# jason-li-831202/Vehicle-CV-ADAS

Hardware: AMD Instinct MI355X
Metric: frames/sec end-to-end (detect+lane+NMS+track) per GPU; conv MFMA util % (higher is better)
Workload: dtype fp16x3

## Files before the change

include/adas_hip.h:

```cpp
#ifndef ADAS_HIP_H
#define ADAS_HIP_H
#include <stddef.h>
#include <stdint.h>

#ifdef __cplusplus
extern "C" {
#endif

typedef enum {
    ADAS_OK = 0,
    ADAS_ERR_INVALID = -1,
    ADAS_ERR_IO = -2,
    ADAS_ERR_FORMAT = -3,
    ADAS_ERR_HIP = -4,
    ADAS_ERR_CAPACITY = -5,
    ADAS_ERR_NO_DEVICE = -6
} adas_status;

const char* adas_last_error(void);
int adas_version(void);
int adas_device_count(void);
int adas_set_device(int index);
int adas_device_pci_bus_id(int index, char* out, int out_len);
int adas_malloc(void** d_ptr, size_t bytes);
int adas_free(void* d_ptr);
int adas_memcpy_h2d(void* d_dst, const void* h_src, size_t bytes);
int adas_memcpy_d2h(void* h_dst, const void* d_src, size_t bytes);
int adas_synchronize(void);
int adas_host_alloc(void** h_ptr, size_t bytes);
int adas_host_free(void* h_ptr);
typedef struct adas_timer adas_timer;
int adas_timer_create(adas_timer** out);
int adas_timer_destroy(adas_timer* t);
int adas_timer_start(adas_timer* t, void* stream);
int adas_timer_stop(adas_timer* t, void* stream);
int adas_timer_elapsed_ms(adas_timer* t, float* ms);

typedef struct adas_engine adas_engine;

#define ADAS_PREC_BF16 0
#define ADAS_PREC_FP32 1
#define ADAS_PREC_FP16 2
#define ADAS_PREC_FP16X3 3

int adas_engine_create(const char* model_path, int precision, int max_batch, adas_engine** out);
int adas_engine_destroy(adas_engine* e);
int adas_engine_input_shape(const adas_engine* e, int64_t dims[4]);
int adas_engine_num_outputs(const adas_engine* e);
int adas_engine_output_shape(const adas_engine* e, int index, int64_t dims[4], int* ndim);
const char* adas_engine_output_name(const adas_engine* e, int index);
int adas_engine_infer_host(adas_engine* e, const float* h_input_nchw, int batch, float* const* h_outputs);
int adas_engine_infer_device(adas_engine* e, const float* d_input_nchw, int batch, void* stream);
int adas_engine_accepts_packed_input(const adas_engine* e);
int adas_engine_precision(const adas_engine* e);
int adas_engine_model_io_half(const adas_engine* e);
int adas_engine_infer_device_packed(adas_engine* e, const uint16_t* d_input_nhwc4, int batch, void* stream);
const float* adas_engine_output_device(const adas_engine* e, int index);
int adas_engine_stats(const adas_engine* e, double* flops_per_frame, double* weight_bytes, int* num_layers);
int adas_engine_profile(adas_engine* e, const float* d_input_nchw, int batch, int iters, float* ms_per_layer,
                        int max_layers, int* num_layers);
int adas_engine_detect_sink_supported(const adas_engine* e);
int adas_engine_detect_sink_shape(const adas_engine* e, int32_t* layout, int32_t* num_anchors, int32_t* num_classes);
int adas_engine_set_detect_sink(adas_engine* e, float* d_best_conf, int32_t* d_best_cls);
int adas_engine_layer_info(const adas_engine* e, int layer, char* name, int name_cap, double* flops, int* kind);
int adas_engine_layer_kernel(const adas_engine* e, int layer, int batch, char* name, int name_cap);
int adas_engine_prepare(adas_engine* e, int batch);
int adas_engine_ml_info(const adas_engine* e, int batch, int32_t* n_launches, int32_t* n_layers, int32_t* n_items);
int adas_engine_ml_status(const adas_engine* e, int batch, uint32_t* error_word);
int adas_engine_launch_count(adas_engine* e, int batch);
int adas_engine_ml_counters(const adas_engine* e, int batch, int launch, uint32_t head16[16]);
typedef struct adas_ml_view {
    uint64_t buf;
    int32_t cs, coff, c, h, w;
} adas_ml_view;
typedef struct adas_ml_layer_desc {
    int32_t kernel, stride, act, res_mode, up_c, halo_bn;
    adas_ml_view x, y, res, up;
} adas_ml_layer_desc;
int adas_debug_ml_plan(const adas_ml_layer_desc* layers, int n_layers, int batch, int precision, int32_t* deps, int32_t* targets,
                       uint64_t* items, int items_cap, int32_t summary[4]);
int adas_debug_conv_route(const adas_ml_layer_desc* layer, int batch, int precision, char* name, int name_cap);
#define ADAS_PLAN_COLS 29
int adas_engine_plan(const adas_engine* e, int64_t* rows, int rows_cap, int32_t* n_ops, uint64_t* weight_bytes);
int adas_debug_engine_plan(const void* tables, size_t bytes, int precision, int max_batch, int64_t* rows, int rows_cap, int32_t* n_ops,
                           uint64_t* weight_bytes);
#define ADAS_LABEL_CAP 96
int adas_engine_schedule(const adas_engine* e, int batch, int32_t* step_of, int32_t* role, int cap, int32_t* n_ops, int32_t* n_steps);
int adas_debug_engine_schedule(const void* tables, size_t bytes, int precision, int max_batch, int batch, int32_t* step_of, int32_t* role,
                               char* labels, int cap, int32_t* n_ops, int32_t* n_steps);
int adas_engine_fetch_activation(adas_engine* e, int layer, int batch, float* h_out_nchw, int64_t dims[4]);

int adas_preprocess_yolo(const uint8_t* d_frames_bgr, int n, int src_h, int src_w, float* d_out_nchw, int dst_h,
                         int dst_w, int keep_ratio, void* stream);
int adas_preprocess_ufld(const uint8_t* d_frames_bgr, int n, int src_h, int src_w, float* d_out_nchw, int in_h,
                         int in_w, double crop_ratio, void* stream);
int adas_preprocess_yolo_packed(const uint8_t* d_frames_bgr, int n, int src_h, int src_w, uint16_t* d_out_nhwc4, int dst_h,
                                int dst_w, int keep_ratio, void* stream);
int adas_preprocess_ufld_packed(const uint8_t* d_frames_bgr, int n, int src_h, int src_w, uint16_t* d_out_nhwc4, int in_h,
                                int in_w, double crop_ratio, void* stream);
int adas_preprocess_yolo_packed_prec(const uint8_t* d_frames_bgr, int n, int src_h, int src_w, uint16_t* d_out_nhwc4, int dst_h,
                                     int dst_w, int keep_ratio, int precision, void* stream);
int adas_preprocess_ufld_packed_prec(const uint8_t* d_frames_bgr, int n, int src_h, int src_w, uint16_t* d_out_nhwc4, int in_h,
                                     int in_w, double crop_ratio, int precision, void* stream);

typedef struct adas_yolo_post adas_yolo_post;

#define ADAS_HEAD_V8 0
#define ADAS_HEAD_V5 1
#define ADAS_HEAD_V5_LITE 2
#define ADAS_NMS_REFERENCE 0
#define ADAS_NMS_GREEDY 1

typedef struct {
    int32_t layout;
    int32_t num_anchors;
    int32_t num_classes;
    int32_t nms_mode;
    double box_score;
    double iou_thr;
    int32_t pad_h, pad_w;
    double ratio_h, ratio_w;
    int32_t max_candidates;
    int32_t reserved;
} adas_yolo_post_params;

int adas_letterbox_params(int src_h, int src_w, int dst_h, int dst_w, int keep_ratio, adas_yolo_post_params* p);

int adas_yolo_post_create(const adas_yolo_post_params* p, int max_batch, adas_yolo_post** out);
int adas_yolo_post_destroy(adas_yolo_post* h);
int adas_yolo_post_set_input_size(adas_yolo_post* h, int in_h, int in_w);
int adas_yolo_post_run(adas_yolo_post* h, const float* d_head, int batch, void* stream);
int adas_yolo_post_scan_views(adas_yolo_post* h, float** d_best_conf, int32_t** d_best_cls);
int adas_yolo_post_run_prescanned(adas_yolo_post* h, const float* d_head, int batch, void* stream);
int adas_yolo_post_profile(adas_yolo_post* h, const float* d_head, int batch, int iters, float ms[2]);

typedef struct {
    int32_t n_found;
    int32_t n_candidates;
    int32_t n_keep;
    int32_t flags;
} adas_yolo_counts;
int adas_yolo_post_fetch(adas_yolo_post* h, int frame, adas_yolo_counts* counts, int32_t* cand_anchor,
                         double* cand_xywh, double* cand_conf, int32_t* cand_cls, int32_t* keep, double* det_xywh,
                         double* det_conf, int32_t* det_cls, int32_t* det_xyxy_int);
int adas_yolo_post_fetch_dets(adas_yolo_post* h, int frame, adas_yolo_counts* counts, int32_t* keep, double* det_xywh,
                              double* det_conf, int32_t* det_cls, int32_t* det_xyxy_int);
int adas_yolo_post_device_views(adas_yolo_post* h, const double** d_xyxy, const double** d_score,
                                const int32_t** d_cls, const int32_t** d_counts);
int adas_yolo_post_capacity(const adas_yolo_post* h, int* max_candidates);
int adas_yolo_post_head_shape(const adas_yolo_post* h, int32_t* layout, int32_t* num_anchors, int32_t* num_classes);

typedef struct adas_effdet_post adas_effdet_post;
typedef struct {
    double box_score;
    int32_t pad_h, pad_w;
    double ratio_h, ratio_w;
    int32_t max_boxes;
    int32_t reserved;
} adas_effdet_post_params;
int adas_effdet_post_create(const adas_effdet_post_params* p, int max_batch, adas_effdet_post** out);
int adas_effdet_post_destroy(adas_effdet_post* h);
int adas_effdet_post_run(adas_effdet_post* h, const float* d_boxes, const int32_t* d_ids, const float* d_confs,
                         const int32_t* h_counts, int batch, void* stream);
int adas_effdet_post_fetch(adas_effdet_post* h, int frame, int32_t* n_keep, float* xywh, float* conf, int32_t* class_id,
                           int32_t* xyxy_int);
typedef struct adas_effdet_tail adas_effdet_tail;
typedef struct {
    int32_t in_h, in_w;
    int32_t num_classes;
    int32_t max_candidates;
    int32_t max_det;
    int32_t reserved;
    double score_thr, iou_thr;
    double anchor_scale;
} adas_effdet_tail_params;
int adas_effdet_tail_create(const adas_effdet_tail_params* p, int max_batch, adas_effdet_tail** out);
int adas_effdet_tail_destroy(adas_effdet_tail* h);
int adas_effdet_tail_run(adas_effdet_tail* h, const float* const* d_reg , const float* const* d_cls , int batch, void* stream);
int adas_effdet_tail_fetch(adas_effdet_tail* h, int frame, int32_t* n_det, float* boxes_xyxy, int32_t* class_id, float* conf,
                           int32_t* n_candidates);
int adas_effdet_tail_device_views(adas_effdet_tail* h, const float** d_boxes, const int32_t** d_ids, const float** d_confs,
                                  const int32_t** d_counts);
int adas_preprocess_effdet(const uint8_t* d_frames_bgr, int n, int src_h, int src_w, float* d_out_nchw, int dst_h, int dst_w,
                           int keep_ratio, void* stream);

typedef struct adas_ufld_decode adas_ufld_decode;
#define ADAS_UFLD_MAX_POINTS 128

typedef struct {
    int32_t grid_row, cls_row, grid_col, cls_col;
    int32_t img_w, img_h;
    int32_t local_width;
    int32_t num_lanes;
    const double* h_row_anchor;
    const double* h_col_anchor;
} adas_ufld_params;

int adas_ufld_decode_create(const adas_ufld_params* p, int max_batch, adas_ufld_decode** out);
int adas_ufld_decode_destroy(adas_ufld_decode* h);
int adas_ufld_decode_run(adas_ufld_decode* h, const float* d_loc_row, const float* d_loc_col,
                         const float* d_exist_row, const float* d_exist_col, size_t stride_loc_row,
                         size_t stride_loc_col, size_t stride_exist_row, size_t stride_exist_col, int batch,
                         void* stream);
int adas_ufld_decode_fetch(adas_ufld_decode* h, int frame, int32_t* points, int32_t* counts, int32_t* detected);
int adas_ufld_decode_upload(adas_ufld_decode* h, int frame, const int32_t* points, const int32_t* counts, const int32_t* detected);

typedef struct {
    int32_t griding_num, cls_num_per_lane;
    int32_t cfg_img_w, cfg_img_h;
    int32_t input_w, input_h;
    int32_t src_w, src_h;
    const double* h_row_anchor;
} adas_ufld1_params;
int adas_ufld1_decode_create(const adas_ufld1_params* p, int max_batch, adas_ufld_decode** out);
int adas_ufld1_decode_set_source_size(adas_ufld_decode* h, int src_w, int src_h);
int adas_ufld_decode_kind(const adas_ufld_decode* h);
int adas_ufld_decode_expected_outputs(const adas_ufld_decode* h, int64_t dims[4][4]);
int adas_ufld1_decode_run(adas_ufld_decode* h, const float* d_out, size_t batch_stride, int batch, void* stream);

typedef struct adas_lane_geometry adas_lane_geometry;
typedef struct {
    int32_t img_h;
    int32_t bird_w, bird_h;
    int32_t adjust_lanes;
    double M[9];
} adas_lane_geometry_params;
typedef struct {
    int32_t area_status;
    int32_t n_area_left, n_area_right;
    int32_t direction;
    int32_t bird_counts[4];
    double curvature;
    double offset;
} adas_lane_geometry_result;
// ... 240 lines not shown
```

vehicle-cv-adas_amd/_lib.py:

```python
import ctypes as C
import os

import numpy as np

HERE = os.path.dirname(os.path.abspath(__file__))
LIB_PATH = os.environ.get("ADAS_LIB") or os.path.join(HERE, "libadas_hip.so")

UFLD_MAX_POINTS = 128
HEAD_V8, HEAD_V5, HEAD_V5_LITE = 0, 1, 2
NMS_REFERENCE, NMS_GREEDY = 0, 1
PREC_BF16, PREC_FP32, PREC_FP16, PREC_FP16X3 = 0, 1, 2, 3
PRECISIONS = {"bf16": PREC_BF16, "fp32": PREC_FP32, "fp16": PREC_FP16, "fp16x3": PREC_FP16X3}


class AdasError(RuntimeError):
    def __init__(self, code, msg):
        super().__init__(f"libadas_hip error {code}: {msg}")
        self.code = code


class YoloPostParams(C.Structure):
    _fields_ = [("layout", C.c_int32), ("num_anchors", C.c_int32), ("num_classes", C.c_int32), ("nms_mode", C.c_int32),
                ("box_score", C.c_double), ("iou_thr", C.c_double), ("pad_h", C.c_int32), ("pad_w", C.c_int32),
                ("ratio_h", C.c_double), ("ratio_w", C.c_double), ("max_candidates", C.c_int32), ("reserved", C.c_int32)]
# ... 9 lines not shown


class EffdetTailParams(C.Structure):
    _fields_ = [("in_h", C.c_int32), ("in_w", C.c_int32), ("num_classes", C.c_int32), ("max_candidates", C.c_int32), ("max_det", C.c_int32),
                ("reserved", C.c_int32), ("score_thr", C.c_double), ("iou_thr", C.c_double), ("anchor_scale", C.c_double)]


class UfldParams(C.Structure):
    _fields_ = [("grid_row", C.c_int32), ("cls_row", C.c_int32), ("grid_col", C.c_int32), ("cls_col", C.c_int32),
                ("img_w", C.c_int32), ("img_h", C.c_int32), ("local_width", C.c_int32), ("num_lanes", C.c_int32),
                ("h_row_anchor", C.c_void_p), ("h_col_anchor", C.c_void_p)]


class Ufld1Params(C.Structure):
    _fields_ = [("griding_num", C.c_int32), ("cls_num_per_lane", C.c_int32), ("cfg_img_w", C.c_int32), ("cfg_img_h", C.c_int32),
                ("input_w", C.c_int32), ("input_h", C.c_int32), ("src_w", C.c_int32), ("src_h", C.c_int32),
                ("h_row_anchor", C.c_void_p)]


class LaneGeometryParams(C.Structure):
    _fields_ = [("img_h", C.c_int32), ("bird_w", C.c_int32), ("bird_h", C.c_int32), ("adjust_lanes", C.c_int32), ("M", C.c_double * 9)]


class LaneGeometryResult(C.Structure):
    _fields_ = [("area_status", C.c_int32), ("n_area_left", C.c_int32), ("n_area_right", C.c_int32), ("direction", C.c_int32),
                ("bird_counts", C.c_int32 * 4), ("curvature", C.c_double), ("offset", C.c_double)]


class WarpParams(C.Structure):
    _fields_ = [("src_h", C.c_int32), ("src_w", C.c_int32), ("dst_h", C.c_int32), ("dst_w", C.c_int32)]


class BirdviewParams(C.Structure):
    _fields_ = [("img_w", C.c_int32), ("img_h", C.c_int32)]


class BirdviewState(C.Structure):
    _fields_ = [("src", C.c_float * 8), ("M", C.c_double * 9), ("M_inv", C.c_double * 9), ("M_warp", C.c_double * 9),
                ("n_updates", C.c_int32), ("n_rejected", C.c_int32)]


BIRDVIEW_MODES = {"Default": 1, "Top": 2, "Bottom": 3}


class AnalysisParams(C.Structure):
    _fields_ = [("focal", C.c_double), ("y_limit", C.c_double), ("distance_thres", C.c_double), ("offset_thres", C.c_double),
                ("curvae_thres", C.c_double), ("calib_curvae_thres", C.c_double), ("calib_frequency", C.c_int32), ("n_classes", C.c_int32),
                ("h_ref_height", C.c_void_p), ("max_points", C.c_int32), ("max_poly", C.c_int32)]


class AnalysisState(C.Structure):
    _fields_ = [("collision_msg", C.c_int32), ("offset_msg", C.c_int32), ("curvature_msg", C.c_int32), ("toggle_status", C.c_int32),
                ("transform_status", C.c_int32), ("oscillator", C.c_int32 * 2), ("counter_offset", C.c_int32), ("counter_curvae", C.c_int32),
                ("counter_birdview", C.c_int32), ("n_collision", C.c_int32), ("n_offset", C.c_int32), ("n_curvature", C.c_int32),
                ("n_nonfinite", C.c_int32), ("collision_record", C.c_double * 5), ("offset_record", C.c_double * 5),
                ("curvature_record", C.c_double * 10), ("direction_record", C.c_int32 * 10)]


class AnalysisInput(C.Structure):
    _fields_ = [("has_point", C.c_int32), ("area", C.c_int32), ("has_offset", C.c_int32), ("has_curvature", C.c_int32), ("direction", C.c_int32),
                ("reserved", C.c_int32), ("distance", C.c_double), ("offset", C.c_double), ("curvature", C.c_double)]


class AnalysisFrame(C.Structure):
    _fields_ = [("n_points", C.c_int32), ("has_collision", C.c_int32), ("collision_x", C.c_int32), ("collision_y", C.c_int32),
                ("collision_d", C.c_double), ("collision_index", C.c_int32), ("collision_msg", C.c_int32), ("offset_msg", C.c_int32),
                ("curvature_msg", C.c_int32), ("toggle_status", C.c_int32), ("transform_status", C.c_int32), ("oscillator", C.c_int32 * 2),
                ("counters", C.c_int32 * 3), ("check", C.c_int32), ("request", C.c_int32), ("flags", C.c_int32)]


ANALYSIS_INPUT_DTYPE = np.dtype([("has_point", "i4"), ("area", "i4"), ("has_offset", "i4"), ("has_curvature", "i4"), ("direction", "i4"),
                                 ("reserved", "i4"), ("distance", "f8"), ("offset", "f8"), ("curvature", "f8")])
ANALYSIS_OVERFLOW, ANALYSIS_NONFINITE, ANALYSIS_TRUNCATED = 1, 2, 4


class OverlayParams(C.Structure):
    _fields_ = [("src_h", C.c_int32), ("src_w", C.c_int32), ("bird_h", C.c_int32), ("bird_w", C.c_int32), ("lane_radius", C.c_int32),
                ("distance_radius", C.c_int32), ("bird_radius", C.c_int32), ("reserved", C.c_int32), ("lane_alpha", C.c_double),
                ("area_alpha", C.c_double), ("lane_colors", (C.c_uint8 * 3) * 4), ("offset_color", C.c_uint8 * 3), ("area_color", C.c_uint8 * 3),
                ("collision_colors", (C.c_uint8 * 3) * 4), ("distance_color", C.c_uint8 * 3), ("pad", C.c_uint8 * 7)]


OVERLAY_LANES, OVERLAY_AREA, OVERLAY_DISTANCE, OVERLAY_BIRD = 1, 2, 4, 8
OVERLAY_STAGES = {"lanes": OVERLAY_LANES, "area": OVERLAY_AREA, "distance": OVERLAY_DISTANCE, "bird": OVERLAY_BIRD}
OVERLAY_POLY_RANGE = 1


class BytetrackParams(C.Structure):
    _fields_ = [("track_thresh", C.c_double), ("match_thresh", C.c_double), ("frame_rate", C.c_double),
                ("track_buffer", C.c_int32), ("max_tracks", C.c_int32), ("max_dets", C.c_int32), ("reserved", C.c_int32)]


class TrackHeader(C.Structure):
    _fields_ = [("frame_id", C.c_int32), ("id_count", C.c_int32), ("n_tracked", C.c_int32), ("n_lost", C.c_int32),
                ("err", C.c_int32), ("pad", C.c_int32 * 3)]


class PipelineDesc(C.Structure):
    _fields_ = [("detector", C.c_void_p), ("lane", C.c_void_p), ("post", C.c_void_p), ("decode", C.c_void_p),
                ("tracker", C.c_void_p), ("n_streams", C.c_int32), ("use_graph", C.c_int32), ("geometry", C.c_void_p),
                ("micro_batch", C.c_int32), ("reserved", C.c_int32)]


class MlView(C.Structure):
    _fields_ = [("buf", C.c_uint64), ("cs", C.c_int32), ("coff", C.c_int32), ("c", C.c_int32), ("h", C.c_int32), ("w", C.c_int32)]


class MlLayerDesc(C.Structure):
    _fields_ = [("kernel", C.c_int32), ("stride", C.c_int32), ("act", C.c_int32), ("res_mode", C.c_int32), ("up_c", C.c_int32), ("halo_bn", C.c_int32),
                ("x", MlView), ("y", MlView), ("res", MlView), ("up", MlView)]


TRACK_DTYPE = np.dtype([("tlwh", "f8", 4), ("score", "f8"), ("track_id", "i4"), ("state", "i4"), ("is_activated", "i4"),
                        ("class_id", "i4"), ("frame_id", "i4"), ("start_frame", "i4"), ("tracklet_len", "i4"), ("traj_len", "i4")])
TRAJECTORY_LEN = 30

_P = C.c_void_p
_SIGS = {
    "adas_last_error": (C.c_char_p, []),
    "adas_version": (C.c_int, []),
    "adas_device_count": (C.c_int, []),
    "adas_set_device": (C.c_int, [C.c_int]),
    "adas_device_pci_bus_id": (C.c_int, [C.c_int, C.c_char_p, C.c_int]),
    "adas_malloc": (C.c_int, [C.POINTER(_P), C.c_size_t]),
    "adas_free": (C.c_int, [_P]),
    "adas_memcpy_h2d": (C.c_int, [_P, _P, C.c_size_t]),
    "adas_memcpy_d2h": (C.c_int, [_P, _P, C.c_size_t]),
    "adas_synchronize": (C.c_int, []),
    "adas_host_alloc": (C.c_int, [C.POINTER(_P), C.c_size_t]),
    "adas_host_free": (C.c_int, [_P]),
    "adas_timer_create": (C.c_int, [C.POINTER(_P)]),
    "adas_timer_destroy": (C.c_int, [_P]),
    "adas_timer_start": (C.c_int, [_P, _P]),
    "adas_timer_stop": (C.c_int, [_P, _P]),
    "adas_timer_elapsed_ms": (C.c_int, [_P, C.POINTER(C.c_float)]),
    "adas_engine_create": (C.c_int, [C.c_char_p, C.c_int, C.c_int, C.POINTER(_P)]),
    "adas_engine_destroy": (C.c_int, [_P]),
    "adas_engine_input_shape": (C.c_int, [_P, C.POINTER(C.c_int64)]),
    "adas_engine_num_outputs": (C.c_int, [_P]),
    "adas_engine_output_shape": (C.c_int, [_P, C.c_int, C.POINTER(C.c_int64), C.POINTER(C.c_int)]),
    "adas_engine_output_name": (C.c_char_p, [_P, C.c_int]),
    "adas_engine_infer_host": (C.c_int, [_P, _P, C.c_int, C.POINTER(_P)]),
    "adas_engine_infer_device": (C.c_int, [_P, _P, C.c_int, _P]),
    "adas_engine_accepts_packed_input": (C.c_int, [_P]),
    "adas_engine_precision": (C.c_int, [_P]),
    "adas_engine_prepare": (C.c_int, [_P, C.c_int]),
    "adas_engine_ml_info": (C.c_int, [_P, C.c_int, C.POINTER(C.c_int32), C.POINTER(C.c_int32), C.POINTER(C.c_int32)]),
    "adas_engine_ml_status": (C.c_int, [_P, C.c_int, C.POINTER(C.c_uint32)]),
    "adas_engine_launch_count": (C.c_int, [_P, C.c_int]),
    "adas_engine_ml_counters": (C.c_int, [_P, C.c_int, C.c_int, C.POINTER(C.c_uint32)]),
    "adas_debug_ml_plan": (C.c_int, [C.POINTER(MlLayerDesc), C.c_int, C.c_int, C.c_int, C.POINTER(C.c_int32), C.POINTER(C.c_int32), C.POINTER(C.c_uint64),
                                     C.c_int, C.POINTER(C.c_int32)]),
    "adas_debug_conv_route": (C.c_int, [C.POINTER(MlLayerDesc), C.c_int, C.c_int, C.c_char_p, C.c_int]),
    "adas_engine_plan": (C.c_int, [_P, C.POINTER(C.c_int64), C.c_int, C.POINTER(C.c_int32), C.POINTER(C.c_uint64)]),
    "adas_debug_engine_plan": (C.c_int, [C.c_char_p, C.c_size_t, C.c_int, C.c_int, C.POINTER(C.c_int64), C.c_int, C.POINTER(C.c_int32), C.POINTER(C.c_uint64)]),
    "adas_engine_schedule": (C.c_int, [_P, C.c_int, C.POINTER(C.c_int32), C.POINTER(C.c_int32), C.c_int, C.POINTER(C.c_int32), C.POINTER(C.c_int32)]),
    "adas_debug_engine_schedule": (C.c_int, [C.c_char_p, C.c_size_t, C.c_int, C.c_int, C.c_int, C.POINTER(C.c_int32), C.POINTER(C.c_int32), C.c_char_p,
                                             C.c_int, C.POINTER(C.c_int32), C.POINTER(C.c_int32)]),
    "adas_engine_model_io_half": (C.c_int, [_P]),
    "adas_engine_infer_device_packed": (C.c_int, [_P, _P, C.c_int, _P]),
    "adas_engine_output_device": (_P, [_P, C.c_int]),
    "adas_engine_stats": (C.c_int, [_P, C.POINTER(C.c_double), C.POINTER(C.c_double), C.POINTER(C.c_int)]),
    "adas_engine_profile": (C.c_int, [_P, _P, C.c_int, C.c_int, _P, C.c_int, C.POINTER(C.c_int)]),
    "adas_engine_layer_info": (C.c_int, [_P, C.c_int, C.c_char_p, C.c_int, C.POINTER(C.c_double), C.POINTER(C.c_int)]),
    "adas_engine_layer_kernel": (C.c_int, [_P, C.c_int, C.c_int, C.c_char_p, C.c_int]),
    "adas_engine_fetch_activation": (C.c_int, [_P, C.c_int, C.c_int, _P, C.POINTER(C.c_int64)]),
    "adas_preprocess_yolo": (C.c_int, [_P, C.c_int, C.c_int, C.c_int, _P, C.c_int, C.c_int, C.c_int, _P]),
    "adas_preprocess_ufld": (C.c_int, [_P, C.c_int, C.c_int, C.c_int, _P, C.c_int, C.c_int, C.c_double, _P]),
    "adas_preprocess_yolo_packed": (C.c_int, [_P, C.c_int, C.c_int, C.c_int, _P, C.c_int, C.c_int, C.c_int, _P]),
    "adas_preprocess_ufld_packed": (C.c_int, [_P, C.c_int, C.c_int, C.c_int, _P, C.c_int, C.c_int, C.c_double, _P]),
    "adas_preprocess_yolo_packed_prec": (C.c_int, [_P, C.c_int, C.c_int, C.c_int, _P, C.c_int, C.c_int, C.c_int, C.c_int, _P]),
    "adas_preprocess_ufld_packed_prec": (C.c_int, [_P, C.c_int, C.c_int, C.c_int, _P, C.c_int, C.c_int, C.c_double, C.c_int, _P]),
    "adas_letterbox_params": (C.c_int, [C.c_int, C.c_int, C.c_int, C.c_int, C.c_int, C.POINTER(YoloPostParams)]),
    "adas_yolo_post_create": (C.c_int, [C.POINTER(YoloPostParams), C.c_int, C.POINTER(_P)]),
    "adas_yolo_post_destroy": (C.c_int, [_P]),
    "adas_yolo_post_set_input_size": (C.c_int, [_P, C.c_int, C.c_int]),
    "adas_yolo_post_run": (C.c_int, [_P, _P, C.c_int, _P]),
    "adas_yolo_post_profile": (C.c_int, [_P, _P, C.c_int, C.c_int, C.POINTER(C.c_float)]),
    "adas_yolo_post_fetch": (C.c_int, [_P, C.c_int, C.POINTER(YoloCounts)] + [_P] * 9),
    "adas_yolo_post_fetch_dets": (C.c_int, [_P, C.c_int, C.POINTER(YoloCounts)] + [_P] * 5),
    "adas_yolo_post_device_views": (C.c_int, [_P] + [C.POINTER(_P)] * 4),
    "adas_yolo_post_scan_views": (C.c_int, [_P, C.POINTER(_P), C.POINTER(_P)]),
    "adas_yolo_post_run_prescanned": (C.c_int, [_P, _P, C.c_int, _P]),
    "adas_engine_detect_sink_supported": (C.c_int, [_P]),
    "adas_engine_detect_sink_shape": (C.c_int, [_P, C.POINTER(C.c_int32), C.POINTER(C.c_int32), C.POINTER(C.c_int32)]),
    "adas_engine_set_detect_sink": (C.c_int, [_P, _P, _P]),
    "adas_pipeline_detect_sink": (C.c_int, [_P]),
    "adas_yolo_post_capacity": (C.c_int, [_P, C.POINTER(C.c_int)]),
    "adas_yolo_post_head_shape": (C.c_int, [_P, C.POINTER(C.c_int32), C.POINTER(C.c_int32), C.POINTER(C.c_int32)]),
    "adas_effdet_post_create": (C.c_int, [C.POINTER(EffdetPostParams), C.c_int, C.POINTER(_P)]),
    "adas_effdet_post_destroy": (C.c_int, [_P]),
    "adas_effdet_post_run": (C.c_int, [_P, _P, _P, _P, _P, C.c_int, _P]),
    "adas_effdet_post_fetch": (C.c_int, [_P, C.c_int, C.POINTER(C.c_int32), _P, _P, _P, _P]),
    "adas_effdet_tail_create": (C.c_int, [C.POINTER(EffdetTailParams), C.c_int, C.POINTER(_P)]),
    "adas_effdet_tail_destroy": (C.c_int, [_P]),
    "adas_effdet_tail_run": (C.c_int, [_P, _P, _P, C.c_int, _P]),
    "adas_effdet_tail_fetch": (C.c_int, [_P, C.c_int, C.POINTER(C.c_int32), _P, _P, _P, C.POINTER(C.c_int32)]),
    "adas_effdet_tail_device_views": (C.c_int, [_P, C.POINTER(_P), C.POINTER(_P), C.POINTER(_P), C.POINTER(_P)]),
    "adas_preprocess_effdet": (C.c_int, [_P, C.c_int, C.c_int, C.c_int, _P, C.c_int, C.c_int, C.c_int, _P]),
    "adas_ufld_decode_create": (C.c_int, [C.POINTER(UfldParams), C.c_int, C.POINTER(_P)]),
    "adas_ufld_decode_destroy": (C.c_int, [_P]),
    "adas_ufld_decode_run": (C.c_int, [_P, _P, _P, _P, _P, C.c_size_t, C.c_size_t, C.c_size_t, C.c_size_t, C.c_int, _P]),
    "adas_ufld_decode_fetch": (C.c_int, [_P, C.c_int, _P, _P, _P]),
    "adas_ufld_decode_upload": (C.c_int, [_P, C.c_int, _P, _P, _P]),
    "adas_ufld1_decode_create": (C.c_int, [C.POINTER(Ufld1Params), C.c_int, C.POINTER(_P)]),
    "adas_ufld1_decode_set_source_size": (C.c_int, [_P, C.c_int, C.c_int]),
    "adas_ufld_decode_kind": (C.c_int, [_P]),
    "adas_ufld_decode_expected_outputs": (C.c_int, [_P, C.POINTER(C.c_int64)]),
    "adas_ufld1_decode_run": (C.c_int, [_P, _P, C.c_size_t, C.c_int, _P]),
    "adas_lane_geometry_create": (C.c_int, [C.POINTER(LaneGeometryParams), C.c_int, C.POINTER(_P)]),
    "adas_lane_geometry_destroy": (C.c_int, [_P]),
    "adas_lane_geometry_set_matrix": (C.c_int, [_P, _P]),
    "adas_lane_geometry_run": (C.c_int, [_P, _P, C.c_int, C.c_int, _P]),
    "adas_lane_geometry_fetch": (C.c_int, [_P, C.c_int, C.POINTER(LaneGeometryResult), _P, _P]),
    "adas_lane_geometry_run_matrices": (C.c_int, [_P, _P, C.c_int, C.c_int, _P, _P]),
    "adas_warp_run_device_matrices": (C.c_int, [_P, _P, _P, _P, C.c_int, _P]),
    "adas_birdview_create": (C.c_int, [C.POINTER(BirdviewParams), C.c_int, C.c_int, C.POINTER(_P)]),
    "adas_birdview_destroy": (C.c_int, [_P]),
    "adas_birdview_reset": (C.c_int, [_P, C.c_int]),
    "adas_birdview_request": (C.c_int, [_P, C.c_int, C.c_int, _P]),
    "adas_birdview_run": (C.c_int, [_P, _P, C.c_int, C.c_int, _P]),
    "adas_birdview_fetch_stream": (C.c_int, [_P, C.c_int, C.POINTER(BirdviewState)]),
    "adas_birdview_fetch_frame": (C.c_int, [_P, C.c_int, _P, _P, C.POINTER(C.c_int32)]),
    "adas_birdview_pending": (C.c_int, [_P, C.c_int, C.POINTER(C.c_int32)]),
    "adas_birdview_device_views": (C.c_int, [_P, C.POINTER(_P), C.POINTER(_P)]),
    "adas_pipeline_attach_birdview": (C.c_int, [_P, _P, _P]),
    "adas_pipeline_attach_analysis": (C.c_int, [_P, _P]),
    "adas_lane_geometry_device_views": (C.c_int, [_P, C.POINTER(_P), C.POINTER(_P), C.POINTER(_P), C.POINTER(C.c_int32)]),
    "adas_analysis_default_params": (C.c_int, [C.POINTER(AnalysisParams)]),
    "adas_analysis_create": (C.c_int, [C.POINTER(AnalysisParams), C.c_int, C.c_int, C.POINTER(_P)]),
    "adas_analysis_destroy": (C.c_int, [_P]),
    "adas_analysis_reset": (C.c_int, [_P, C.c_int]),
    "adas_analysis_run": (C.c_int, [_P, _P, _P, _P, C.c_int, C.c_int, _P]),
    "adas_analysis_run_arrays": (C.c_int, [_P, _P, _P, _P, C.c_int, _P, C.c_int, _P, _P, _P, C.c_int, C.c_int, _P]),
    "adas_analysis_run_inputs": (C.c_int, [_P, _P, C.c_int, C.c_int, _P]),
    "adas_analysis_fetch_stream": (C.c_int, [_P, C.c_int, C.POINTER(AnalysisState)]),
    "adas_analysis_fetch_frame": (C.c_int, [_P, C.c_int, C.POINTER(AnalysisFrame)]),
    "adas_analysis_fetch_points": (C.c_int, [_P, C.c_int, _P, _P, C.c_int]),
    "adas_pipeline_request_transform": (C.c_int, [_P, C.c_int, C.c_int]),
    "adas_overlay_default_params": (C.c_int, [C.POINTER(OverlayParams)]),
    "adas_overlay_create": (C.c_int, [C.POINTER(OverlayParams), C.c_int, C.POINTER(_P)]),
    "adas_overlay_destroy": (C.c_int, [_P]),
    "adas_overlay_set_style": (C.c_int, [_P, C.POINTER(OverlayParams)]),
    "adas_overlay_run": (C.c_int, [_P, _P, _P, _P, _P, _P, _P, C.c_int, C.c_int, C.c_int, _P]),
    "adas_overlay_run_arrays": (C.c_int, [_P, _P, _P, _P, _P, _P, C.c_int, _P, _P, _P, _P, _P, C.c_int, _P, _P, _P, _P, C.c_int, C.c_int, _P]),
    "adas_overlay_fetch": (C.c_int, [_P, C.c_int, _P]),
    "adas_overlay_device_view": (C.c_int, [_P, C.POINTER(_P)]),
    "adas_overlay_fetch_flags": (C.c_int, [_P, C.c_int, C.POINTER(C.c_int32)]),
    "adas_pipeline_attach_overlay": (C.c_int, [_P, _P]),
    "adas_pipeline_set_overlay_stages": (C.c_int, [_P, C.c_int]),
    "adas_warp_create": (C.c_int, [C.POINTER(WarpParams), C.c_int, C.POINTER(_P)]),
    "adas_warp_destroy": (C.c_int, [_P]),
    "adas_warp_set_matrix": (C.c_int, [_P, C.c_int, _P, C.c_int]),
    "adas_warp_run": (C.c_int, [_P, _P, _P, C.c_int, _P]),
    "adas_warp_fetch": (C.c_int, [_P, C.c_int, _P]),
    "adas_warp_device_view": (C.c_int, [_P, C.POINTER(_P)]),
    "adas_bytetrack_create": (C.c_int, [C.POINTER(BytetrackParams), C.c_int, C.POINTER(_P)]),
    "adas_bytetrack_destroy": (C.c_int, [_P]),
    "adas_bytetrack_reset": (C.c_int, [_P, C.c_int]),
    "adas_bytetrack_update_host": (C.c_int, [_P, C.c_int, _P, _P, _P, C.c_int]),
    "adas_bytetrack_update_device": (C.c_int, [_P, _P, _P, _P, _P, C.c_int, C.c_int, C.c_int, C.c_int, _P]),
    "adas_bytetrack_update_device_frames": (C.c_int, [_P, _P, _P, _P, _P, C.c_int, C.c_int, C.c_int, C.c_int, C.c_int, _P]),
    "adas_bytetrack_fetch": (C.c_int, [_P, C.c_int, C.POINTER(TrackHeader), _P, C.c_int]),
    "adas_bytetrack_fetch_trajectories": (C.c_int, [_P, C.c_int, _P, _P, C.c_int, C.POINTER(C.c_int32)]),
    "adas_bytetrack_reserve_frames": (C.c_int, [_P, C.c_int, C.c_int]),
    "adas_bytetrack_fetch_frame": (C.c_int, [_P, C.c_int, C.c_int, C.POINTER(TrackHeader), _P, C.c_int]),
    "adas_pipeline_create": (C.c_int, [C.POINTER(PipelineDesc), C.POINTER(_P)]),
    "adas_pipeline_destroy": (C.c_int, [_P]),
    "adas_pipeline_step": (C.c_int, [_P, _P, _P]),
    "adas_pipeline_step_frames": (C.c_int, [_P, _P, C.c_int, C.c_int, C.c_double]),
    "adas_pipeline_step_frames_host": (C.c_int, [_P, _P, C.c_int, C.c_int, C.c_double]),
    "adas_pipeline_wait_upload": (C.c_int, [_P]),
    "adas_pipeline_sync": (C.c_int, [_P]),
    "adas_pipeline_timings": (C.c_int, [_P, C.POINTER(C.c_float)]),
}

_lib = None


def exported_symbols():
    return sorted(_SIGS)


def lib():
    global _lib
    if _lib is None:
        if not os.path.exists(LIB_PATH):
            raise RuntimeError(f"{LIB_PATH} is not built; run `python vehicle-cv-adas_amd/build.py` "
                               "(hipcc --offload-arch=gfx950). There is no CPU fallback.")
        L = C.CDLL(LIB_PATH)
        for name, (res, args) in _SIGS.items():
            fn = getattr(L, name)
            fn.restype = res
            fn.argtypes = args
        _lib = L
    return _lib


def check(code):
    if code != 0:
        raise AdasError(code, lib().adas_last_error().decode("utf-8", "replace"))
    return code


def ptr(a):
    return None if a is None else a.ctypes.data_as(C.c_void_p)
# ... 92 lines not shown
```

vehicle-cv-adas_amd/csrc/conv_halo8_x3.hip:

```cpp
#include "kernels.h"
#include "elem16.h"
#include <stdlib.h>
#include <string.h>
#include <type_traits>

namespace adas {

typedef __attribute__((ext_vector_type(4))) float yf32x4;
typedef __attribute__((ext_vector_type(4))) uint32_t yu32x4;
typedef __attribute__((ext_vector_type(2))) uint32_t yu32x2;
typedef __attribute__((address_space(3))) void* ylds_vp;

struct H8XDev {
    const void* in;
    const void* wgt;
    const float* bias;
    void* out;
    const void* res;
    uint32_t in_bytes, wgt_bytes, out_bytes, res_bytes;
    int in_cs, in_coff, cin, H, W;
    int out_cs, out_coff, cout;
    int res_cs, res_coff, res_mode;
    int nck;
    int SW, NS, TPS, WW;
    uint32_t mg_ww, mg_sw;
    uint32_t mg_img, mg_tps, mg_upt;
    int ntiles, tiles8, ncb, cpw;
};

constexpr int X8_THR = 512;
constexpr int X8_BM = 256;
constexpr int X8_MAXPIX = 640;
constexpr int X8_WIN = X8_MAXPIX * 64;
constexpr int X8_TAP = 2 * 64 * 64;
constexpr int X8_WR = 2 * X8_WIN;
constexpr int X8_LDS = X8_WR + 9 * X8_TAP;
constexpr int X8_NWP = X8_MAXPIX / 16 / 8;
constexpr int X8_SLAB = 9 * 64 * 64;
constexpr uint32_t X8_OOB = 0xF0000000u;
constexpr int X8_SLOTS = 32;

__host__ __device__ constexpr int x8_look(int mode) { return mode == 2 ? 6 : 4; }

template <int N>
__device__ __forceinline__ void x8_wait_vm() {
    asm volatile("s_waitcnt vmcnt(%0)" ::"n"(N) : "memory");
}

template <int ACT>
__device__ __forceinline__ float x8_act(float v) {
    if (ACT == ACT_SILU) return x3_silu(v);
    if (ACT == ACT_RELU) return fmaxf(v, 0.0f);
    if (ACT == ACT_LEAKY) return fmaxf(v, 0.1f * v);
    return v;
}

typedef __attribute__((ext_vector_type(2))) float yf32x2;
template <int ACT>
__device__ __forceinline__ yf32x2 x8_act2(yf32x2 v) {
    if (ACT == ACT_RELU) return __builtin_elementwise_max(v, yf32x2{0.0f, 0.0f});
    return yf32x2{x8_act<ACT>(v[0]), x8_act<ACT>(v[1])};
}
__device__ __forceinline__ yf32x2 x8_join2(uint32_t h, uint32_t l) {
    return __builtin_convertvector(__builtin_bit_cast(e_f16x2, l), yf32x2) * kX3Down + __builtin_convertvector(__builtin_bit_cast(e_f16x2, h), yf32x2);
}
__device__ __forceinline__ void x8_hi_mode(bool flush) {
    if (flush) __builtin_amdgcn_s_setreg((unsigned short)(1 | (6 << 6) | (1 << 11)), 0u);
    else __builtin_amdgcn_s_setreg((unsigned short)(1 | (6 << 6) | (1 << 11)), 3u);
}
__device__ __forceinline__ uint32_t x8_cvt_hi2(yf32x2 v) {
    uint32_t h;
    asm volatile("v_cvt_pk_f16_f32 %0, %1, %2" : "=v"(h) : "v"(v[0]), "v"(v[1]));
    return h;
}
__device__ __forceinline__ uint32_t x8_lo2(yf32x2 v, uint32_t h) {
    const yf32x2 d = (v - __builtin_convertvector(__builtin_bit_cast(e_f16x2, h), yf32x2)) * kX3Up;
    return __builtin_bit_cast(uint32_t, __builtin_convertvector(d, e_f16x2));
}

__host__ __device__ constexpr int x8_issued(int k) { return 1 + ((k >= 1 && k <= X8_NWP) ? 1 : 0); }
__host__ __device__ constexpr int x8_allow(int mode, int k) {
    return mode == 2 ? x8_issued(k) + x8_issued(k - 1) + x8_issued(k - 2)
                     : x8_issued(k) + x8_issued((k + 8) % 9) + x8_issued((k + 7) % 9);
}
#ifndef ADAS_H8X_RES_TAP
#define ADAS_H8X_RES_TAP 0
#endif
constexpr int X8_RES_TAP = ADAS_H8X_RES_TAP;
#ifdef ADAS_H8X_NARROW_ST
constexpr int X8_NBIAS = 2, X8_NRES = 16;
#else
constexpr int X8_NBIAS = 2, X8_NRES = 8;
#endif

#ifdef ADAS_H8X_PROF
__device__ unsigned long long g_h8x_prof[256][32];
#define H8XP(i)                                     \
    if (lane == 0 && grp == 0) {                    \
        const unsigned long long t__ = clock64();   \
        pacc__[i] += t__ - tprev__;                 \
        tprev__ = t__;                              \
    }
#else
#define H8XP(i)
#endif

__host__ __device__ constexpr int x8s_issued(bool lo, int k, int nwp) { return ((lo ? k >= 3 : (k >= 0 && k < 3)) ? 1 : 0) + ((k >= 1 && k <= nwp) ? 1 : 0); }
__host__ __device__ constexpr int x8s_allow(bool lo, int k, int nwp) { return x8s_issued(lo, k, nwp) + x8s_issued(lo, k - 1, nwp) + x8s_issued(lo, k - 2, nwp); }

template <int ACT, int MODE, bool LH, bool SH, int NWP>
__global__ __launch_bounds__(X8_THR, 1) void conv_h8x3_kernel(H8XDev a) {
    static_assert(!SH || (MODE == 2 && !LH), "shared weight tiles: one barrier per tap row, whole tiles");
    static_assert(NWP >= 1 && NWP <= X8_NWP && (SH || NWP == X8_NWP), "window pieces per wave");
    Fp16::enter();
    typedef Fp16::vec8 hvec8;
    constexpr int LOOK = x8_look(MODE);
    extern __shared__ __attribute__((aligned(16))) uint8_t lds8[];

    const int tid = threadIdx.x, lane = tid & 63;
    const int wave = __builtin_amdgcn_readfirstlane(tid >> 6);
    const int lrow = lane & 15, kg = lane >> 4;
    const int hb = wave >> 2, grp = wave & 3;
    const int xcd = blockIdx.x & 7, slot = blockIdx.x >> 3, nslot = gridDim.x >> 3;
    int tiles_here = a.ntiles - xcd * a.tiles8;
    tiles_here = tiles_here < 0 ? 0 : (tiles_here > a.tiles8 ? a.tiles8 : tiles_here);
    const int upt = a.ncb / a.cpw;
    const int units_here = tiles_here * upt;
    if (slot >= units_here) return;

    __amdgpu_buffer_rsrc_t rin = __builtin_amdgcn_make_buffer_rsrc((void*)a.in, 0, a.in_bytes, 0x00020000);
    __amdgpu_buffer_rsrc_t rwg = __builtin_amdgcn_make_buffer_rsrc((void*)a.wgt, 0, a.wgt_bytes, 0x00020000);
    __amdgpu_buffer_rsrc_t rout = __builtin_amdgcn_make_buffer_rsrc((void*)a.out, 0, a.out_bytes, 0x00020000);
    __amdgpu_buffer_rsrc_t rres = __builtin_amdgcn_make_buffer_rsrc((void*)(a.res_mode != RES_NONE ? a.res : a.out), 0,
                                                                    a.res_mode != RES_NONE ? a.res_bytes : 0u, 0x00020000);
    const int per_img = a.NS * a.TPS;
    const int gsw[4] = {0, 2, 3, 1};
    const uint32_t wlane = (uint32_t)((lane >> 2) * 64 + (((lane & 3) ^ gsw[(lane >> 4) & 3]) << 4));
    const uint32_t wpiece = (uint32_t)((lane & 3) ^ (((lane >> 4) & 1) << 1)) << 5;
    const uint32_t wrd = (uint32_t)(X8_WR + hb * 4096 + lrow * 64 + ((kg ^ gsw[(lrow >> 2) & 3]) << 4));
    const uint32_t wlane_h = (uint32_t)((lane >> 2) * 64 + (((lane & 3) ^ gsw[(((lane >> 4) & 1) + 2 * (grp & 1)) & 3]) << 4));
    const uint32_t wdst_h = (uint32_t)(X8_WR + hb * 4096 + 2048 + grp * 512);
#ifdef ADAS_H8X_NARROW_ST
    const uint32_t ch_lane = (uint32_t)((hb * 4 + (kg >> 1)) * 32 + (kg & 1) * 8);
#else
    const uint32_t ch_lane = (uint32_t)((hb * 4 + (kg >> 1)) * 32 + (kg & 1) * 16);
#endif
    const bool has_res = a.res_mode != RES_NONE;

    struct Tile {
        int img, sx0, p0, y_first;
    };
    auto decode = [&](int u) {
        Tile t;
        int tile = xcd * a.tiles8 + (upt == 1 ? u : (int)__umulhi((uint32_t)u, a.mg_upt));
        t.img = per_img == 1 ? tile : (int)__umulhi((uint32_t)tile, a.mg_img);
        tile -= t.img * per_img;
        const int strip = a.TPS == 1 ? tile : (int)__umulhi((uint32_t)tile, a.mg_tps);
        t.sx0 = strip * a.SW;
        t.p0 = (tile - strip * a.TPS) * X8_BM;
        t.y_first = (int)(((uint32_t)t.p0 * a.mg_sw) >> 20);
        return t;
    };
    auto win_offset = [&](const Tile& t, int i) {
        const int y_lastp = (int)(((uint32_t)(t.p0 + X8_BM - 1) * a.mg_sw) >> 20);
        const int npix = (y_lastp - t.y_first + 3) * a.WW;
        const int pix = (wave + 8 * i) * 16 + (lane >> 2);
        const int wy = (int)(((uint32_t)pix * a.mg_ww) >> 20), wx = pix - wy * a.WW;
        const int iy = t.y_first - 1 + wy, ix = t.sx0 - 1 + wx;
        const bool ok = pix < npix && (unsigned)iy < (unsigned)a.H && (unsigned)ix < (unsigned)a.W;
        const uint32_t off = ((uint32_t)((t.img * a.H + iy) * a.W + ix) * (uint32_t)a.in_cs + (uint32_t)a.in_coff) * 4u + wpiece;
        const uint32_t m = 0u - (uint32_t)ok;
        return (off & m) | (X8_OOB & ~m);
    };
    auto tap00 = [&](const Tile& t, int j) {
        const int p = t.p0 + (grp * 4 + j) * 16 + lrow;
        const int y = (int)(((uint32_t)p * a.mg_sw) >> 20), xs = p - y * a.SW;
        return (uint32_t)((((y - t.y_first) * a.WW + xs) << 6) | (kg << 4));
    };
    auto tap_offset = [&](uint32_t ap64, int t) {
        const uint32_t v = ap64 + (uint32_t)(((t / 3) * a.WW + (t % 3)) << 6);
        return v ^ ((v >> 3) & 0x20u);
    };
    auto out_pixel = [&](const Tile& t, int j) {
        const int p = t.p0 + (grp * 4 + j) * 16 + lrow;
        const int y = (int)(((uint32_t)p * a.mg_sw) >> 20), x = t.sx0 + (p - y * a.SW);
        return (y < a.H && x < a.W) ? (uint32_t)((t.img * a.H + y) * a.W + x) : X8_OOB;
    };
    auto wgt_base = [&](int cb) { return (uint32_t)(((2 * cb + hb) * a.nck) * X8_SLAB + grp * 1024); };
    auto load_bias = [&](int cb, float4* b) {
#pragma unroll
        for (int i = 0; i < 2; ++i) b[i] = *reinterpret_cast<const float4*>(a.bias + cb * 64 + hb * 32 + i * 16 + kg * 4);
    };

    auto first_cb = [&](int u) { return upt == 1 ? 0 : (u - (int)__umulhi((uint32_t)u, a.mg_upt) * upt) * a.cpw; };
    int ti = slot, cb = first_cb(slot), cbi = 0;
    Tile cur = decode(ti);
    uint32_t gcur[X8_NWP], gnxt[X8_NWP];
    uint32_t xoff[4][9];
    uint32_t po[4];
#pragma unroll
    for (int i = 0; i < NWP; ++i) gcur[i] = win_offset(cur, i);
#pragma unroll
    for (int j = 0; j < 4; ++j) {
        const uint32_t ap64 = tap00(cur, j);
#pragma unroll
        for (int t = 0; t < 9; ++t) xoff[j][t] = tap_offset(ap64, t);
        po[j] = out_pixel(cur, j);
    }
    uint32_t wcur = wgt_base(cb);
    int par = 0;
    float4 biasn[2];
    load_bias(cb, biasn);

#pragma unroll
    for (int i = 0; i < NWP; ++i)
        __builtin_amdgcn_raw_ptr_buffer_load_lds(rin, (ylds_vp)(lds8 + (wave + 8 * i) * 1024), 16, gcur[i], 0, 0, 0);
#pragma unroll
    for (int t = 0; t < LOOK; ++t)
        __builtin_amdgcn_raw_ptr_buffer_load_lds(rwg, (ylds_vp)(lds8 + X8_WR + t * X8_TAP + wave * 1024), 16, wlane, wcur + t * 4096, 0, 0);
    yf32x4 acc[4][4];
#pragma unroll
    for (int j = 0; j < 4; ++j) {
#pragma unroll
        for (int i = 0; i < 2; ++i) {
            acc[i][j] = yf32x4{biasn[i].x, biasn[i].y, biasn[i].z, biasn[i].w};
            acc[i + 2][j] = yf32x4{0.f, 0.f, 0.f, 0.f};
        }
    }
    x8_wait_vm<0>();
    __builtin_amdgcn_s_barrier();
    if (MODE == 1 && hb) __builtin_amdgcn_s_barrier();
#ifdef ADAS_H8X_PROF
    unsigned long long tprev__ = clock64();
    unsigned long long pacc__[16] = {0, 0, 0, 0, 0, 0, 0, 0, 0, 0, 0, 0, 0, 0, 0, 0};
    int nit__ = 0;
#endif

    for (;;) {
        H8XP(0)
        const bool newtile = cbi + 1 == a.cpw;
        const bool has_next = !newtile || ti + nslot < units_here;
        const int cbn = newtile ? first_cb(has_next ? ti + nslot : ti) : cb + 1;
        const uint32_t ch0 = (uint32_t)(cb * 256) + ch_lane;
#ifndef ADAS_H8X_NO_TRIM
        const bool wave_on = cb * 64 + hb * 32 < a.cout;
#else
        constexpr bool wave_on = true;
#endif
        Tile nxt = cur;
        uint32_t wnxt_item = 0, apn[4] = {0, 0, 0, 0};
        yu32x4 rraw[4][2];

        auto chunk = [&](auto last_c, auto lo_c, const int c) {
            constexpr bool lastc = decltype(last_c)::value;
            constexpr bool islo = decltype(lo_c)::value;
            if (lastc) {
                if (newtile && has_next) nxt = decode(ti + nslot);
                if (!has_next) nxt.y_first = a.H + 4;
                wnxt_item = wgt_base(cbn);
#pragma unroll
                for (int j = 0; j < 4; ++j) apn[j] = tap00(nxt, j);
            } else {
#pragma unroll
                for (int i = 0; i < NWP; ++i) gcur[i] += islo ? 112u : 16u;
            }
            const uint32_t wthis = wcur + (uint32_t)c * X8_SLAB;
            const uint32_t wnext = lastc ? wnxt_item : wthis + X8_SLAB;
            const uint32_t winr = (uint32_t)(((par + c) & 1) * X8_WIN), winw = X8_WIN - winr;
            auto tap = [&](auto kk_c) {
                constexpr int kk = decltype(kk_c)::value;
                if (lastc && kk == X8_RES_TAP) load_bias(cbn, biasn);
                if (lastc && kk == X8_RES_TAP && has_res) {
#pragma unroll
                    for (int j = 0; j < 4; ++j) {
                        const uint32_t ro = po[j] == X8_OOB ? X8_OOB : (po[j] * (uint32_t)a.res_cs + (uint32_t)a.res_coff) * 4u + ch0;
#pragma unroll
                        for (int i = 0; i < 2; ++i) {
#ifdef ADAS_H8X_NARROW_ST
                            const uint32_t ri = (cb * 64 + hb * 32 + i * 16 + kg * 4 < a.cout) ? ro + i * 64 : X8_OOB;
                            const yu32x2 rh = __builtin_bit_cast(yu32x2, __builtin_amdgcn_raw_buffer_load_b64(rres, ri, 0, 0));
                            const yu32x2 rl = __builtin_bit_cast(yu32x2, __builtin_amdgcn_raw_buffer_load_b64(rres, ri + 16, 0, 0));
                            rraw[j][i] = yu32x4{rh.x, rh.y, rl.x, rl.y};
#else
                            const uint32_t ri = (cb * 64 + hb * 32 + i * 16 + (kg >> 1) * 8 < a.cout) ? ro + i * 64 : X8_OOB;
                            rraw[j][i] = __builtin_bit_cast(yu32x4, __builtin_amdgcn_raw_buffer_load_b128(rres, ri, 0, 0));
#endif
                        }
                    }
                }
                hvec8 wf[4], xf[4];
                if (wave_on) {
#pragma unroll
                    for (int i = islo ? 2 : 0; i < 4; ++i) wf[i] = *reinterpret_cast<const hvec8*>(lds8 + wrd + kk * X8_TAP + ((SH && islo) ? i - 2 : i) * 1024);
#pragma unroll
                    for (int j = 0; j < 4; ++j) xf[j] = *reinterpret_cast<const hvec8*>(lds8 + xoff[j][kk] + winr);
                }
                if constexpr (SH) {
                    if constexpr (islo ? kk >= 3 : kk < 3) {
                        constexpr int kt = (kk + 6) % 9;
                        const uint32_t src = (islo ? wnext : wthis) + (uint32_t)kt * 4096u;
                        __builtin_amdgcn_raw_ptr_buffer_load_lds(rwg, (ylds_vp)(lds8 + X8_WR + kt * X8_TAP + wave * 1024), 16, wlane, src, 0, 0);
                    }
                } else {
                    constexpr int kt = (kk + LOOK) % 9;
                    constexpr bool tgt_lo = (kk + LOOK < 9) ? islo : !islo;
                    const uint32_t src = (kk + LOOK < 9 ? wthis : wnext) + (uint32_t)kt * 4096u;
                    if (LH && tgt_lo) {
                        if (lane < 32)
                            __builtin_amdgcn_raw_ptr_buffer_load_lds(rwg, (ylds_vp)(lds8 + wdst_h + kt * X8_TAP), 16, wlane_h, src + 2048u - (uint32_t)grp * 512u, 0, 0);
                    } else {
                        __builtin_amdgcn_raw_ptr_buffer_load_lds(rwg, (ylds_vp)(lds8 + X8_WR + kt * X8_TAP + wave * 1024), 16, wlane, src, 0, 0);
                    }
                }
                if constexpr (kk >= 1 && kk <= NWP)
                    __builtin_amdgcn_raw_ptr_buffer_load_lds(rin, (ylds_vp)(lds8 + winw + (wave + 8 * (kk - 1)) * 1024), 16, lastc ? gnxt[kk - 1] : gcur[kk - 1], 0, 0, 0);
                constexpr bool sync_here = MODE != 2 || kk % 3 == 2;
                constexpr int allow = SH ? x8s_allow(islo, kk, NWP) : x8_allow(MODE, kk);
                constexpr bool with_res = kk >= X8_RES_TAP && (MODE == 2 ? kk / 3 == X8_RES_TAP / 3 : kk < X8_RES_TAP + 3);
                auto counted_wait = [&]() {
                    if (sync_here && (c > 0 || kk >= 3)) {
                        if (lastc && with_res && has_res) x8_wait_vm<allow + X8_NBIAS + X8_NRES>();
                        else if (lastc && with_res) x8_wait_vm<allow + X8_NBIAS>();
                        else x8_wait_vm<allow>();
                    }
                };
#ifndef ADAS_H8X_WAIT_LAST
                counted_wait();
#else
                if (MODE == 1) counted_wait();
#endif
                if (MODE == 1) {
                    __builtin_amdgcn_sched_barrier(0);
                    __builtin_amdgcn_s_barrier();
                    __builtin_amdgcn_sched_barrier(0);
                }
                __builtin_amdgcn_s_setprio(1);
                if (lastc) {
#pragma unroll
                    for (int j = 0; j < 4; ++j) xoff[j][kk] = tap_offset(apn[j], kk);
                    if constexpr (kk < NWP) gnxt[kk] = win_offset(nxt, kk);
                }
                if (wave_on) {
#pragma unroll
                    for (int i = islo ? 2 : 0; i < 4; ++i)
#pragma unroll
                        for (int j = 0; j < 4; ++j) acc[i][j] = Fp16::mfma(wf[i], xf[j], acc[i][j]);
                }
                if (lastc) {
#pragma unroll
                    for (int g = 0; g < (islo ? 8 : 16); ++g) {
                        __builtin_amdgcn_sched_group_barrier(0x008, 1, 0);
                        __builtin_amdgcn_sched_group_barrier(0x006, 6, 0);
                    }
                }
                __builtin_amdgcn_s_setprio(0);
                if (sync_here) {
                    __builtin_amdgcn_sched_barrier(0);
#ifdef ADAS_H8X_WAIT_LAST
                    if (MODE != 1) counted_wait();
#endif
                    __builtin_amdgcn_s_barrier();
                    __builtin_amdgcn_sched_barrier(0);
                }
            };
            tap(std::integral_constant<int, 0>{}); tap(std::integral_constant<int, 1>{}); tap(std::integral_constant<int, 2>{});
            tap(std::integral_constant<int, 3>{}); tap(std::integral_constant<int, 4>{}); tap(std::integral_constant<int, 5>{});
            tap(std::integral_constant<int, 6>{}); tap(std::integral_constant<int, 7>{}); tap(std::integral_constant<int, 8>{});
#ifdef ADAS_H8X_PROF
            if (lastc) { H8XP(3) } else if (islo) { H8XP(2) } else { H8XP(1) }
#endif
        };
        for (int c = 0; c + 1 < a.nck; ++c) {
            if (c & 1) chunk(std::false_type{}, std::true_type{}, c);
            else chunk(std::false_type{}, std::false_type{}, c);
        }
        chunk(std::true_type{}, std::true_type{}, a.nck - 1);

        __builtin_amdgcn_s_waitcnt(0x0F70);
        H8XP(4)
#if !defined(ADAS_H8X_SCALAR_EPI) && !defined(ADAS_H8X_NARROW_ST)
        auto write_out = [&](auto rm_c) {
            constexpr int RM = decltype(rm_c)::value;
            yf32x2 val[4][2][2];
#pragma unroll
            for (int j = 0; j < 4; ++j)
#pragma unroll
                for (int i = 0; i < 2; ++i) {
                    yf32x2 v0 = yf32x2{acc[i + 2][j][0], acc[i + 2][j][1]} * kX3Down + yf32x2{acc[i][j][0], acc[i][j][1]};
                    yf32x2 v1 = yf32x2{acc[i + 2][j][2], acc[i + 2][j][3]} * kX3Down + yf32x2{acc[i][j][2], acc[i][j][3]};
                    if (RM != RES_NONE) {
                        const auto q0 = __builtin_amdgcn_permlane16_swap(rraw[j][i].x, rraw[j][i].z, false, false);
                        const auto q1 = __builtin_amdgcn_permlane16_swap(rraw[j][i].y, rraw[j][i].w, false, false);
                        const yf32x2 r0 = x8_join2(q0[0], q0[1]), r1 = x8_join2(q1[0], q1[1]);
                        if (RM == RES_BEFORE_ACT) { v0 = x8_act2<ACT>(v0 + r0); v1 = x8_act2<ACT>(v1 + r1); }
                        else { v0 = x8_act2<ACT>(v0) + r0; v1 = x8_act2<ACT>(v1) + r1; }
                    } else {
                        v0 = x8_act2<ACT>(v0); v1 = x8_act2<ACT>(v1);
                    }
                    val[j][i][0] = v0; val[j][i][1] = v1;
                    acc[i][j] = yf32x4{biasn[i].x, biasn[i].y, biasn[i].z, biasn[i].w};
                    acc[i + 2][j] = yf32x4{0.f, 0.f, 0.f, 0.f};
                }
            uint32_t hw[4][2][2];
            x8_hi_mode(true);
#pragma unroll
            for (int j = 0; j < 4; ++j)
#pragma unroll
                for (int i = 0; i < 2; ++i) {
                    hw[j][i][0] = x8_cvt_hi2(val[j][i][0]);
                    hw[j][i][1] = x8_cvt_hi2(val[j][i][1]);
                }
            x8_hi_mode(false);
#pragma unroll
            for (int j = 0; j < 4; ++j) {
                const uint32_t oo = po[j] == X8_OOB ? X8_OOB : (po[j] * (uint32_t)a.out_cs + (uint32_t)a.out_coff) * 4u + ch0;
#pragma unroll
                for (int i = 0; i < 2; ++i) {
                    const uint32_t oi = (cb * 64 + hb * 32 + i * 16 + (kg >> 1) * 8 < a.cout) ? oo + i * 64 : X8_OOB;
                    const uint32_t l0 = x8_lo2(val[j][i][0], hw[j][i][0]), l1 = x8_lo2(val[j][i][1], hw[j][i][1]);
                    const auto s0 = __builtin_amdgcn_permlane16_swap(hw[j][i][0], l0, false, false);
                    const auto s1 = __builtin_amdgcn_permlane16_swap(hw[j][i][1], l1, false, false);
                    __builtin_amdgcn_raw_buffer_store_b128(yu32x4{s0[0], s1[0], s0[1], s1[1]}, rout, oi, 0, 0);
                }
            }
        };
#else
        auto write_out = [&](auto rm_c) {
            constexpr int RM = decltype(rm_c)::value;
#pragma unroll
            for (int j = 0; j < 4; ++j) {
                const uint32_t oo = po[j] == X8_OOB ? X8_OOB : (po[j] * (uint32_t)a.out_cs + (uint32_t)a.out_coff) * 4u + ch0;
#pragma unroll
                for (int i = 0; i < 2; ++i) {
#ifdef ADAS_H8X_NARROW_ST
                    const uint32_t oi = (cb * 64 + hb * 32 + i * 16 + kg * 4 < a.cout) ? oo + i * 64 : X8_OOB;
#else
                    const uint32_t oi = (cb * 64 + hb * 32 + i * 16 + (kg >> 1) * 8 < a.cout) ? oo + i * 64 : X8_OOB;
#endif
                    float v[4];
#pragma unroll
                    for (int e = 0; e < 4; ++e) v[e] = acc[i][j][e] + acc[i + 2][j][e] * kX3Down;
                    if (RM != RES_NONE) {
#ifdef ADAS_H8X_NARROW_ST
                        const uint32_t wh0 = rraw[j][i].x, wh1 = rraw[j][i].y, wl0 = rraw[j][i].z, wl1 = rraw[j][i].w;
#else
                        const auto q0 = __builtin_amdgcn_permlane16_swap(rraw[j][i].x, rraw[j][i].z, false, false);
                        const auto q1 = __builtin_amdgcn_permlane16_swap(rraw[j][i].y, rraw[j][i].w, false, false);
                        const uint32_t wh0 = q0[0], wl0 = q0[1], wh1 = q1[0], wl1 = q1[1];
#endif
                        const e_f16x2 h0 = __builtin_bit_cast(e_f16x2, wh0);
                        const e_f16x2 h1 = __builtin_bit_cast(e_f16x2, wh1);
                        const e_f16x2 l0 = __builtin_bit_cast(e_f16x2, wl0);
                        const e_f16x2 l1 = __builtin_bit_cast(e_f16x2, wl1);
                        const float r[4] = {x3_join(h0[0], l0[0]), x3_join(h0[1], l0[1]), x3_join(h1[0], l1[0]), x3_join(h1[1], l1[1])};
#pragma unroll
                        for (int e = 0; e < 4; ++e) v[e] = RM == RES_BEFORE_ACT ? x8_act<ACT>(v[e] + r[e]) : x8_act<ACT>(v[e]) + r[e];
                    } else {
#pragma unroll
                        for (int e = 0; e < 4; ++e) v[e] = x8_act<ACT>(v[e]);
                    }
                    e_f16x2 h0, h1, l0, l1;
                    _Float16 h, l;
                    x3_split(v[0], h, l); h0[0] = h; l0[0] = l;
                    x3_split(v[1], h, l); h0[1] = h; l0[1] = l;
                    x3_split(v[2], h, l); h1[0] = h; l1[0] = l;
                    x3_split(v[3], h, l); h1[1] = h; l1[1] = l;
#ifdef ADAS_H8X_NARROW_ST
                    __builtin_amdgcn_raw_buffer_store_b64(yu32x2{__builtin_bit_cast(uint32_t, h0), __builtin_bit_cast(uint32_t, h1)}, rout, oi, 0, 0);
                    __builtin_amdgcn_raw_buffer_store_b64(yu32x2{__builtin_bit_cast(uint32_t, l0), __builtin_bit_cast(uint32_t, l1)}, rout, oi + 16, 0, 0);
#else
                    {
                        const auto s0 = __builtin_amdgcn_permlane16_swap(__builtin_bit_cast(uint32_t, h0), __builtin_bit_cast(uint32_t, l0), false, false);
                        const auto s1 = __builtin_amdgcn_permlane16_swap(__builtin_bit_cast(uint32_t, h1), __builtin_bit_cast(uint32_t, l1), false, false);
                        __builtin_amdgcn_raw_buffer_store_b128(yu32x4{s0[0], s1[0], s0[1], s1[1]}, rout, oi, 0, 0);
                    }
#endif
                    acc[i][j] = yf32x4{biasn[i].x, biasn[i].y, biasn[i].z, biasn[i].w};
                    acc[i + 2][j] = yf32x4{0.f, 0.f, 0.f, 0.f};
                }
            }
        };
#endif
        if (a.res_mode == RES_NONE) write_out(std::integral_constant<int, RES_NONE>{});
        else if (a.res_mode == RES_BEFORE_ACT) write_out(std::integral_constant<int, RES_BEFORE_ACT>{});
        else write_out(std::integral_constant<int, RES_AFTER_ACT>{});
        H8XP(5)
#ifdef ADAS_H8X_PROF
        ++nit__;
#endif

        if (!has_next) break;
        if (newtile) {
            ti += nslot;
            cur = nxt;
#pragma unroll
            for (int j = 0; j < 4; ++j) po[j] = out_pixel(cur, j);
        }
        cb = cbn;
        cbi = newtile ? 0 : cbi + 1;
#pragma unroll
        for (int i = 0; i < NWP; ++i) gcur[i] = gnxt[i];
        wcur = wnxt_item;
        par = (par + a.nck) & 1;
    }
    if (MODE == 1 && !hb) __builtin_amdgcn_s_barrier();
#ifdef ADAS_H8X_PROF
    if (lane == 0 && grp == 0) {
        unsigned long long* b__ = g_h8x_prof[blockIdx.x & 255];
        for (int i__ = 0; i__ < 16; ++i__)
            if (i__ != 7) atomicAdd(&b__[i__ + 16 * hb], pacc__[i__]);
        atomicAdd(&b__[7 + 16 * hb], (unsigned long long)nit__);
    }
#endif
}

#ifdef ADAS_H8X_PROF
extern "C" int adas_debug_h8x_prof(unsigned long long* out32, int reset) {
    static unsigned long long h[256][32];
    if (out32) {
        if (hipMemcpyFromSymbol(h, HIP_SYMBOL(g_h8x_prof), sizeof(h)) != hipSuccess) return -1;
        for (int i = 0; i < 32; ++i) {
            out32[i] = 0;
            for (int b = 0; b < 256; ++b) out32[i] += h[b][i];
        }
    }
    if (reset) {
        memset(h, 0, sizeof(h));
        if (hipMemcpyToSymbol(HIP_SYMBOL(g_h8x_prof), h, sizeof(h)) != hipSuccess) return -1;
    }
    return 0;
}
#endif

static int x8_mode() {
    static int v = -1;
    if (v < 0) {
        const char* e = getenv("ADAS_HALO8_X3");
        v = e ? atoi(e) : 1;
    }
    return v;
}

static int x8_policy() {
    static int v = -1;
    if (v < 0) {
        const char* e = getenv("ADAS_H8X_PLAN");
        v = e ? atoi(e) : 1;
    }
    return v;
}
static bool x8_plan(int Ho, int Wo, HaloPlan* pl) { return plan_halo(Ho, Wo, 1, pl, X8_MAXPIX, 0, x8_policy()); }

static double x8_min_fill() {
    static double v = -1.0;
    if (v < 0) { const char* e = getenv("ADAS_H8X_MIN_FILL"); v = e ? atof(e) : 0.6; if (!(v > 0.0 && v <= 1.0)) v = 0.6; }
    return v;
}
static int x8_blocks_per_unit(long tiles8, int ncb) {
    for (int cpw = ncb; cpw >= 1; --cpw) {
        if (ncb % cpw) continue;
        const long units8 = tiles8 * (ncb / cpw), rounds = (units8 + X8_SLOTS - 1) / X8_SLOTS;
        if (units8 >= X8_SLOTS && (double)units8 / (double)(rounds * X8_SLOTS) >= x8_min_fill()) return cpw;
    }
    if (tiles8 * ncb >= 12 && tiles8 * ncb < X8_SLOTS) return 1;
    return 0;
}

static int x8_cin_pad(int cin) { return (cin + 31) / 32 * 32; }
static int x8_cout_pad(int cout) { return (cout + 63) / 64 * 64; }
bool halo8_x3_shape_ok(int kh, int kw, int stride, int pad, const TView& in, const TView& out) {
    if (!x8_mode()) return false;
    if (kh != 3 || kw != 3 || stride != 1 || pad != 1) return false;
    if (in.f32 || out.f32 || out.h != in.h || out.w != in.w) return false;
    if ((out.c & 7) || (in.c & 7) || in.c < 16) return false;
    if ((in.cs & 7) || (in.coff & 7) || (out.cs & 7) || (out.coff & 7)) return false;
    if ((double)in.c * out.c < 0.5 * (double)x8_cin_pad(in.c) * x8_cout_pad(out.c)) return false;
    HaloPlan pl;
    return x8_plan(out.h, out.w, &pl) && pl.eff >= 0.6 && pl.maxpix <= X8_MAXPIX;
}
size_t halo8_x3_weight_bytes(int cout, int cin) { return (size_t)(x8_cout_pad(cout) / 32) * (size_t)(2 * (x8_cin_pad(cin) / 32)) * X8_SLAB; }

bool halo8_x3_applicable(const ConvArgs& a) {
    const TView &in = a.in, &out = a.out, &res = a.res;
    const int n = a.n, res_mode = a.res_mode;
    if (!halo8_x3_shape_ok(a.kh, a.kw, a.stride, a.pad, in, out)) return false;
    if (res_mode != RES_NONE && ((res.cs & 7) || (res.coff & 7) || res.f32)) return false;
    if ((double)n * in.h * in.w * in.cs * 4.0 >= (double)X8_OOB || (double)n * out.h * out.w * out.cs * 4.0 >= (double)X8_OOB) return false;
    if (res_mode != RES_NONE && (double)n * out.h * out.w * res.cs * 4.0 >= (double)X8_OOB) return false;
    if ((double)halo8_x3_weight_bytes(out.c, in.c) >= (double)X8_OOB) return false;
    HaloPlan pl;
    if (!x8_plan(out.h, out.w, &pl)) return false;
    const long ntiles = (long)n * pl.NS * pl.TPS, tiles8 = (ntiles + 7) / 8;
    if (ntiles * (x8_cout_pad(out.c) / 64) * pl.NS * pl.TPS >= (1L << 32)) return false;
    return x8_blocks_per_unit(tiles8, x8_cout_pad(out.c) / 64) > 0;
}

__global__ void pack_weights_h8x3_kernel(const float* __restrict__ src, uint16_t* __restrict__ dst, int cout, int cin, int nck, size_t total) {
    for (size_t i = (size_t)blockIdx.x * blockDim.x + threadIdx.x; i < total; i += (size_t)gridDim.x * blockDim.x) {
        const int k = (int)(i & 31);
        size_t r = i >> 5;
        const int row = (int)(r & 63); r >>= 6;
        const int tap = (int)(r % 9); r /= 9;
        const int ck = (int)(r % nck);
        const size_t blk = r / nck;
        const size_t co = blk * 32 + (row & 31);
        const int ci = (ck >> 1) * 32 + k;
        const float w = (co < (size_t)cout && ci < cin) ? src[(co * 9 + tap) * cin + ci] : 0.0f;
        _Float16 h, l;
        x3_split(w, h, l);
        const bool cross = row >= 32, lo_chunk = (ck & 1) != 0;
        const _Float16 v = lo_chunk ? (cross ? h : (_Float16)0.0f) : (cross ? l : h);
        dst[i] = __builtin_bit_cast(uint16_t, v);
    }
}
hipError_t launch_pack_weights_h8x3(const float* src, void* dst, int cout, int cin, hipStream_t st) {
    if ((cout & 7) || (cin & 7)) return hipErrorInvalidValue;
    const size_t total = halo8_x3_weight_bytes(cout, cin) / 2;
    const int blocks = (int)((total + 255) / 256 < 8192 ? (total + 255) / 256 : 8192);
    hipLaunchKernelGGL(pack_weights_h8x3_kernel, dim3(blocks), dim3(256), 0, st, src, (uint16_t*)dst, cout, cin, 2 * (x8_cin_pad(cin) / 32), total);
    return hipGetLastError();
}

static bool x8_lhalf() {
    static int v = -1;
    if (v < 0) {
        const char* e = getenv("ADAS_H8X_LHALF");
        v = e ? atoi(e) : 1;
    }
    return v != 0;
}

static bool x8_share() {
    static int v = -1;
    if (v < 0) {
        const char* e = getenv("ADAS_H8X_SHARE");
        v = e ? atoi(e) : 1;
    }
    return v != 0;
}

template <int NWP>
static hipError_t x8_launch_sh(const H8XDev& d, int act, dim3 grid, hipStream_t st) {
    static bool attr_done = false;
    if (!attr_done) {
        (void)hipFuncSetAttribute((const void*)conv_h8x3_kernel<ACT_NONE, 2, false, true, NWP>, hipFuncAttributeMaxDynamicSharedMemorySize, 160 * 1024);
        (void)hipFuncSetAttribute((const void*)conv_h8x3_kernel<ACT_SILU, 2, false, true, NWP>, hipFuncAttributeMaxDynamicSharedMemorySize, 160 * 1024);
        (void)hipFuncSetAttribute((const void*)conv_h8x3_kernel<ACT_RELU, 2, false, true, NWP>, hipFuncAttributeMaxDynamicSharedMemorySize, 160 * 1024);
        (void)hipFuncSetAttribute((const void*)conv_h8x3_kernel<ACT_LEAKY, 2, false, true, NWP>, hipFuncAttributeMaxDynamicSharedMemorySize, 160 * 1024);
        attr_done = true;
    }
    if (act == ACT_SILU) hipLaunchKernelGGL((conv_h8x3_kernel<ACT_SILU, 2, false, true, NWP>), grid, dim3(X8_THR), X8_LDS, st, d);
    else if (act == ACT_RELU) hipLaunchKernelGGL((conv_h8x3_kernel<ACT_RELU, 2, false, true, NWP>), grid, dim3(X8_THR), X8_LDS, st, d);
    else if (act == ACT_LEAKY) hipLaunchKernelGGL((conv_h8x3_kernel<ACT_LEAKY, 2, false, true, NWP>), grid, dim3(X8_THR), X8_LDS, st, d);
    else hipLaunchKernelGGL((conv_h8x3_kernel<ACT_NONE, 2, false, true, NWP>), grid, dim3(X8_THR), X8_LDS, st, d);
    return hipGetLastError();
}

template <int MODE, bool LH>
static hipError_t x8_launch(const H8XDev& d, int act, dim3 grid, hipStream_t st) {
    static bool attr_done = false;
    if (!attr_done) {
        (void)hipFuncSetAttribute((const void*)conv_h8x3_kernel<ACT_NONE, MODE, LH, false, X8_NWP>, hipFuncAttributeMaxDynamicSharedMemorySize, 160 * 1024);
        (void)hipFuncSetAttribute((const void*)conv_h8x3_kernel<ACT_SILU, MODE, LH, false, X8_NWP>, hipFuncAttributeMaxDynamicSharedMemorySize, 160 * 1024);
        (void)hipFuncSetAttribute((const void*)conv_h8x3_kernel<ACT_RELU, MODE, LH, false, X8_NWP>, hipFuncAttributeMaxDynamicSharedMemorySize, 160 * 1024);
        (void)hipFuncSetAttribute((const void*)conv_h8x3_kernel<ACT_LEAKY, MODE, LH, false, X8_NWP>, hipFuncAttributeMaxDynamicSharedMemorySize, 160 * 1024);
        attr_done = true;
    }
    if (act == ACT_SILU) hipLaunchKernelGGL((conv_h8x3_kernel<ACT_SILU, MODE, LH, false, X8_NWP>), grid, dim3(X8_THR), X8_LDS, st, d);
    else if (act == ACT_RELU) hipLaunchKernelGGL((conv_h8x3_kernel<ACT_RELU, MODE, LH, false, X8_NWP>), grid, dim3(X8_THR), X8_LDS, st, d);
    else if (act == ACT_LEAKY) hipLaunchKernelGGL((conv_h8x3_kernel<ACT_LEAKY, MODE, LH, false, X8_NWP>), grid, dim3(X8_THR), X8_LDS, st, d);
    else hipLaunchKernelGGL((conv_h8x3_kernel<ACT_NONE, MODE, LH, false, X8_NWP>), grid, dim3(X8_THR), X8_LDS, st, d);
    return hipGetLastError();
}

hipError_t launch_conv_halo8_x3(const ConvArgs& a, hipStream_t st) {
    HaloPlan pl;
    if (!a.wgt_h8x3 || !halo8_x3_applicable(a) || !x8_plan(a.out.h, a.out.w, &pl)) return hipErrorInvalidValue;
    {
        static int sw = -1;
        if (sw < 0) { const char* e = getenv("ADAS_H8X_SW"); sw = e ? atoi(e) : 0; }
        HaloPlan alt;
        if (sw > 0 && plan_halo_sw(a.out.h, a.out.w, 1, sw, X8_MAXPIX, &alt) && alt.eff >= 0.6) {
            const long nt = (long)a.n * alt.NS * alt.TPS;
            if (x8_blocks_per_unit((nt + 7) / 8, x8_cout_pad(a.out.c) / 64) > 0) pl = alt;
        }
    }
    H8XDev d;
    d.in = a.in.p; d.wgt = a.wgt_h8x3; d.bias = a.bias; d.out = a.out.p; d.res = a.res.p;
    d.in_cs = a.in.cs; d.in_coff = a.in.coff; d.cin = a.in.c; d.H = a.in.h; d.W = a.in.w;
    d.out_cs = a.out.cs; d.out_coff = a.out.coff; d.cout = a.out.c;
    d.res_cs = a.res.cs; d.res_coff = a.res.coff; d.res_mode = a.res_mode;
    d.nck = 2 * (x8_cin_pad(a.in.c) / 32);
    d.in_bytes = (uint32_t)((size_t)a.n * a.in.h * a.in.w * a.in.cs * 4);
    d.wgt_bytes = (uint32_t)halo8_x3_weight_bytes(a.out.c, a.in.c);
    d.out_bytes = (uint32_t)((size_t)a.n * a.out.h * a.out.w * a.out.cs * 4);
    d.res_bytes = a.res_mode != RES_NONE ? (uint32_t)((size_t)a.n * a.out.h * a.out.w * a.res.cs * 4) : 0u;
    d.SW = pl.SW; d.NS = pl.NS; d.TPS = pl.TPS; d.WW = pl.WW;
    d.mg_ww = pl.mg_ww; d.mg_sw = pl.mg_sw;
    d.mg_img = (uint32_t)(((1ull << 32) + (uint64_t)(pl.NS * pl.TPS) - 1) / (uint64_t)(pl.NS * pl.TPS));
    d.mg_tps = (uint32_t)(((1ull << 32) + (uint64_t)pl.TPS - 1) / (uint64_t)pl.TPS);
    d.ntiles = a.n * pl.NS * pl.TPS;
    d.tiles8 = (d.ntiles + 7) / 8;
    d.ncb = x8_cout_pad(a.out.c) / 64;
    d.cpw = x8_blocks_per_unit(d.tiles8, d.ncb);
    if (d.cpw <= 0) return hipErrorInvalidValue;
    const int upt = d.ncb / d.cpw;
    d.mg_upt = (uint32_t)(((1ull << 32) + (uint64_t)upt - 1) / (uint64_t)upt);
    const int units8 = d.tiles8 * upt;
    static int max_slots = -1;
    if (max_slots < 0) { const char* e = getenv("ADAS_H8X_SLOTS"); max_slots = e ? atoi(e) : X8_SLOTS; if (max_slots < 8 || max_slots > 4096) max_slots = X8_SLOTS; }
    const int slots = units8 < max_slots ? units8 : max_slots;
    dim3 grid(8 * slots);
    const int forced = x8_mode();
    const bool pingpong = forced == 3;
    if (x8_share() && forced != 3) {
        const int nwp = (pl.maxpix + 127) / 128;
        if (nwp <= 3) return x8_launch_sh<3>(d, a.act, grid, st);
        if (nwp == 4) return x8_launch_sh<4>(d, a.act, grid, st);
        return x8_launch_sh<5>(d, a.act, grid, st);
    }
    if (x8_lhalf()) return pingpong ? x8_launch<1, true>(d, a.act, grid, st) : x8_launch<2, true>(d, a.act, grid, st);
    return pingpong ? x8_launch<1, false>(d, a.act, grid, st) : x8_launch<2, false>(d, a.act, grid, st);
}

}
```

vehicle-cv-adas_amd/csrc/engine.cpp:

```cpp
#include "engine.h"
#include <string.h>
#include <string>
#include <vector>

using namespace adas;

int adas::free_engine(adas_engine* e) {
    if (!e) return ADAS_OK;
    for (auto& kv : e->schedules) free_schedule(&kv.second);
    e->schedules.clear();
    for (auto& b : e->bufs)
        if (b.d && b.alias_of < 0) (void)hipFree(b.d);
    if (e->d_weights) (void)hipFree(e->d_weights);
    if (e->d_input) (void)hipFree(e->d_input);
    for (auto& ev : e->events)
        if (ev) (void)hipEventDestroy(ev);
    delete e;
    return ADAS_OK;
}

extern "C" {

int adas_engine_destroy(adas_engine* e) { return free_engine(e); }

// ... 232 lines not shown
        (void)hipGetLastError();
        return ADAS_ERR_HIP;
    }
    return ADAS_OK;
}

int run_step(adas_engine* e, const Step& step, const float* d_in, int batch, hipStream_t st, bool packed_in) {
    if (step.kind == Step::OP) return engine_run_op(e, step, d_in, batch, st, packed_in);
    const hipError_t err = step.kind == Step::GROUP ? ml_group_launch(step.group, st) : ml_launch(step.plan, st);
    if (err == hipSuccess) return ADAS_OK;
    if (step.kind == Step::GROUP) set_error("layers %d..%d: grouped launch failed: %s", step.members.front(), step.members.back(), hipGetErrorString(err));
    else
        set_error("layers %d..%d (%s ...): multi-layer launch failed: %s", step.members.front(), step.members.back(), e->ops[step.lead].name.c_str(),
                  hipGetErrorString(err));
    (void)hipGetLastError();
    return ADAS_ERR_HIP;
}

bool stream_capturing(hipStream_t st) {
    hipStreamCaptureStatus cs = hipStreamCaptureStatusNone;
    if (hipStreamIsCapturing(st, &cs) != hipSuccess) { (void)hipGetLastError(); return false; }
    return cs != hipStreamCaptureStatusNone;
}

}

int adas::engine_forward(adas_engine* e, const float* d_in, int batch, hipStream_t st, bool packed_in) {
    if (!e->schedules.count(batch) && !stream_capturing(st)) {
        int rc = engine_prepare(e, batch);
        if (rc != ADAS_OK) return rc;
    }
    Schedule local;
    for (const Step& step : schedule_at(e, batch, &local).steps) {
        int rc = run_step(e, step, d_in, batch, st, packed_in);
        if (rc != ADAS_OK) return rc;
    }
    return ADAS_OK;
}

extern "C" {

int adas_engine_infer_device(adas_engine* e, const float* d_input, int batch, void* stream) {
    ADAS_REQUIRE(e && d_input && batch > 0 && batch <= e->max_batch, ADAS_ERR_INVALID, "adas_engine_infer_device: bad argument (batch %d, max %d)", batch,
                 e ? e->max_batch : 0);
    e->last = (hipStream_t)stream;
    return engine_forward(e, d_input, batch, (hipStream_t)stream);
}

int adas_engine_prepare(adas_engine* e, int batch) {
    ADAS_REQUIRE(e && batch > 0 && batch <= e->max_batch, ADAS_ERR_INVALID, "adas_engine_prepare: bad argument (batch %d, max %d)", batch, e ? e->max_batch : 0);
    return engine_prepare(e, batch);
}
static std::vector<const Step*> ml_steps(const adas_engine* e, int batch) {
    std::vector<const Step*> v;
    auto it = e->schedules.find(batch);
    if (it != e->schedules.end())
        for (auto& st : it->second.steps)
            if (st.kind == Step::ML) v.push_back(&st);
    return v;
}
int adas_engine_ml_info(const adas_engine* e, int batch, int32_t* n_launches, int32_t* n_layers, int32_t* n_items) {
    ADAS_REQUIRE(e && batch > 0, ADAS_ERR_INVALID, "adas_engine_ml_info: bad argument");
    int nl = 0, ni = 0, ns = 0;
    for (const Step* st : ml_steps(e, batch)) { ++ns; nl += (int)st->members.size(); ni += st->ml_items; }
    if (n_launches) *n_launches = ns;
    if (n_layers) *n_layers = nl;
    if (n_items) *n_items = ni;
    return ADAS_OK;
}
int adas_engine_ml_status(const adas_engine* e, int batch, uint32_t* error_word) {
    ADAS_REQUIRE(e && error_word, ADAS_ERR_INVALID, "adas_engine_ml_status: bad argument");
    *error_word = 0;
    for (const Step* st : ml_steps(e, batch)) {
        unsigned w = 0;
        ADAS_REQUIRE(ml_plan_status(st->plan, &w) == 0, ADAS_ERR_HIP, "adas_engine_ml_status: could not read the control block");
        if (w) {
            *error_word = w;
            set_error("multi-layer launch of layers %d..%d: a dependency wait timed out (item %u)", st->members.front(), st->members.back(), w - 1);
            return ADAS_ERR_HIP;
        }
    }
    return ADAS_OK;
}
int adas_engine_ml_counters(const adas_engine* e, int batch, int launch, uint32_t head16[16]) {
    ADAS_REQUIRE(e && head16, ADAS_ERR_INVALID, "adas_engine_ml_counters: bad argument");
    const std::vector<const Step*> steps = ml_steps(e, batch);
    ADAS_REQUIRE(launch >= 0 && launch < (int)steps.size(), ADAS_ERR_INVALID, "adas_engine_ml_counters: no multi-layer launch %d at batch %d", launch, batch);
    unsigned w = 0;
    ADAS_REQUIRE(ml_plan_status(steps[launch]->plan, &w, head16) == 0, ADAS_ERR_HIP, "adas_engine_ml_counters: could not read the control block");
    return ADAS_OK;
}
int adas_engine_launch_count(adas_engine* e, int batch) {
    if (!e || batch <= 0 || batch > e->max_batch) return -1;
    Schedule local;
    return (int)schedule_at(e, batch, &local).steps.size();
}

static ConvArgs conv_args_of_desc(const adas_ml_layer_desc& d, int batch, int precision) {
    auto view = [](const adas_ml_view& v) {
        TView t;
        t.p = (void*)(uintptr_t)v.buf; t.cs = v.cs; t.coff = v.coff; t.c = v.c; t.h = v.h; t.w = v.w; t.f32 = 0;
        return t;
    };
    ConvArgs a;
    a.in = view(d.x); a.out = view(d.y);
    if (d.res_mode != RES_NONE) a.res = view(d.res);
    else { a.res = a.out; a.res.p = nullptr; }
    a.wgt = (const void*)(uintptr_t)0x1000; a.bias = (const float*)(uintptr_t)0x1000;
    a.n = batch; a.kh = a.kw = d.kernel == CONV_PW ? 1 : 3; a.stride = d.stride; a.pad = d.kernel == CONV_PW ? 0 : 1; a.act = d.act; a.res_mode = d.res_mode;
    a.k = a.kh * a.kw * a.in.c; a.kpad = (a.kh * a.kw * ((a.in.c + 31) / 32 * 32) + 31) / 32 * 32; a.m = batch * a.out.h * a.out.w; a.max_n = batch; a.prec = precision;
    a.halo_bn = d.halo_bn;
    if (d.up_c > 0) { a.up = view(d.up); a.up_c = d.up_c; }
    return a;
}

int adas_debug_ml_plan(const adas_ml_layer_desc* layers, int n_layers, int batch, int precision, int32_t* deps, int32_t* targets, uint64_t* items,
                       int items_cap, int32_t summary[4]) {
    ADAS_REQUIRE(layers && n_layers > 0 && batch > 0 && deps && targets && summary, ADAS_ERR_INVALID, "adas_debug_ml_plan: bad argument");
    std::vector<ConvArgs> ls;
    std::vector<int> ks;
    for (int i = 0; i < n_layers; ++i) {
        ls.push_back(conv_args_of_desc(layers[i], batch, precision));
        ks.push_back(layers[i].kernel);
    }
    std::string why;
    MlPlanInfo info;
    MlPlan* pl = ml_plan_create(ls, ks, precision, &why, &info, true);
    ADAS_REQUIRE(pl, ADAS_ERR_INVALID, "adas_debug_ml_plan: %s", why.c_str());
    ml_plan_destroy(pl);
    for (int i = 0; i < n_layers; ++i)
        for (int k = 0; k < ML_MAX_DEPS; ++k) {
            deps[i * ML_MAX_DEPS + k] = k < (int)info.deps[i].size() ? info.deps[i][k] : -1;
            targets[i * ML_MAX_DEPS + k] = k < (int)info.targets[i].size() ? info.targets[i][k] : 0;
        }
    summary[0] = info.n_items; summary[1] = info.grid; summary[2] = (int32_t)info.lds; summary[3] = info.order;
    if (items) {
        ADAS_REQUIRE(items_cap >= info.n_items, ADAS_ERR_CAPACITY, "adas_debug_ml_plan: %d items, room for %d", info.n_items, items_cap);
        for (int k = 0; k < info.n_items; ++k) items[k] = info.item_words[k];
    }
    return ADAS_OK;
}

int adas_debug_conv_route(const adas_ml_layer_desc* layer, int batch, int precision, char* name, int name_cap) {
    ADAS_REQUIRE(layer && batch > 0 && precision >= PREC_BF16 && precision <= PREC_X3 && name && name_cap > 0, ADAS_ERR_INVALID,
                 "adas_debug_conv_route: bad argument");
    ConvArgs a = conv_args_of_desc(*layer, batch, precision);
    const ConvPlan pl = plan_conv(precision, a.kh, a.kw, a.stride, a.pad, a.max_n, a.res_mode, a.in, a.out);
    a.kpad = pl.kpad;
    if (wants_x3h8_packing(precision, pl.kernel, a.kh, a.kw, a.stride, a.pad, a.res_mode, a.in, a.out)) a.wgt_h8x3 = (const void*)(uintptr_t)0x1000;
    snprintf(name, name_cap, "%s", conv_kernel_name(a));
    return ADAS_OK;
}

int adas_engine_precision(const adas_engine* e) { return e ? e->prec : -1; }
int adas_engine_model_io_half(const adas_engine* e) { return e ? (int)((e->hdr.in_cpad >> 16) & 1u) : 0; }

int adas_engine_accepts_packed_input(const adas_engine* e) {
    return (e && e->prec != PREC_X3 && e->ops.size() >= 2 && e->ops[0].skip && e->ops[1].kernel == CONV_STEM) ? 1 : 0;
}

int adas_engine_infer_device_packed(adas_engine* e, const uint16_t* d_input_nhwc4, int batch, void* stream) {
    ADAS_REQUIRE(e && d_input_nhwc4 && batch > 0 && batch <= e->max_batch, ADAS_ERR_INVALID, "adas_engine_infer_device_packed: bad argument");
    ADAS_REQUIRE(adas_engine_accepts_packed_input(e), ADAS_ERR_INVALID,
                 "this engine's first layer is not the fused stem (fp32 mode or ADAS_NO_STEM): feed the fp32 NCHW tensor instead");
    e->last = (hipStream_t)stream;
    return engine_forward(e, reinterpret_cast<const float*>(d_input_nhwc4), batch, (hipStream_t)stream, true);
}

const float* adas_engine_output_device(const adas_engine* e, int index) {
    if (!e || index < 0 || index >= (int)e->outs.size()) return nullptr;
    const EngOut& o = e->outs[index];
    return (const float*)e->bufs[o.buf].d + o.offset;
}

int adas_engine_infer_host(adas_engine* e, const float* h_input, int batch, float* const* h_outputs) {
    ADAS_REQUIRE(e && h_input && h_outputs && batch > 0 && batch <= e->max_batch, ADAS_ERR_INVALID, "adas_engine_infer_host: bad argument");
    size_t in_bytes = (size_t)batch * e->hdr.in_c * e->hdr.in_h * e->hdr.in_w * 4;
    ADAS_HIP_TRY(hipMemcpyAsync(e->d_input, h_input, in_bytes, hipMemcpyHostToDevice, 0));
    int rc = adas_engine_infer_device(e, e->d_input, batch, nullptr);
    if (rc != ADAS_OK) return rc;
    for (size_t i = 0; i < e->outs.size(); ++i) {
        const EngOut& o = e->outs[i];
        const EngBuf& b = e->bufs[o.buf];
        size_t frame_stride = (size_t)b.h * b.w * b.c;
        ADAS_HIP_TRY(hipMemcpy2DAsync(h_outputs[i], o.elems * 4, (const float*)b.d + o.offset, frame_stride * 4, o.elems * 4, batch,
                                      hipMemcpyDeviceToHost, 0));
    }
    ADAS_HIP_TRY(hipStreamSynchronize(0));
    if (e->mode == adas_engine::ML) {
        uint32_t w = 0;
        int rc = adas_engine_ml_status(e, batch, &w);
        if (rc != ADAS_OK) return rc;
    }
    return ADAS_OK;
}

int adas_engine_profile(adas_engine* e, const float* d_input, int batch, int iters, float* ms_per_layer, int max_layers, int* num_layers) {
    ADAS_REQUIRE(e && d_input && batch > 0 && batch <= e->max_batch && iters > 0 && ms_per_layer, ADAS_ERR_INVALID, "adas_engine_profile: bad argument");
    const int n = (int)e->ops.size();
    ADAS_REQUIRE(max_layers >= n, ADAS_ERR_INVALID, "need room for %d layers", n);
    {
        int rc = engine_prepare(e, batch);
        if (rc != ADAS_OK) return rc;
    }
    const std::vector<Step>& steps = e->schedules.at(batch).steps;
    const size_t n_ev = (steps.size() > 8 ? steps.size() : 8) + 1;
    while (e->events.size() < n_ev) {
        hipEvent_t ev = nullptr;
        ADAS_HIP_TRY(hipEventCreate(&ev));
        e->events.push_back(ev);
    }
    for (int i = 0; i < n; ++i) ms_per_layer[i] = 0.f;
    float marker_ms = 0.f;
    {
        const int reps = 8;
        for (int r = 0; r <= reps; ++r) ADAS_HIP_TRY(hipEventRecord(e->events[r], 0));
        ADAS_HIP_TRY(hipStreamSynchronize(0));
        float lo = 1e30f;
        for (int r = 1; r < reps; ++r) {
            float ms = 0.f;
            ADAS_HIP_TRY(hipEventElapsedTime(&ms, e->events[r], e->events[r + 1]));
            lo = ms < lo ? ms : lo;
        }
        marker_ms = lo < 1e29f ? lo : 0.f;
    }
    for (int it = 0; it < iters; ++it) {
        ADAS_HIP_TRY(hipEventRecord(e->events[0], 0));
        for (size_t k = 0; k < steps.size(); ++k) {
            int rc = run_step(e, steps[k], d_input, batch, 0, false);
            if (rc != ADAS_OK) return rc;
            ADAS_HIP_TRY(hipEventRecord(e->events[k + 1], 0));
        }
        ADAS_HIP_TRY(hipStreamSynchronize(0));
        for (size_t k = 0; k < steps.size(); ++k) {
            float ms = 0.f;
            ADAS_HIP_TRY(hipEventElapsedTime(&ms, e->events[k], e->events[k + 1]));
            ms -= marker_ms;
            ms_per_layer[steps[k].lead] += (ms > 0.f ? ms : 0.f) / (float)iters;
        }
    }
    if (num_layers) *num_layers = n;
    return ADAS_OK;
}

int adas_engine_fetch_activation(adas_engine* e, int layer, int batch, float* h_out, int64_t dims[4]) {
    ADAS_REQUIRE(e && layer >= 0 && layer < (int)e->ops.size() && batch > 0 && batch <= e->max_batch, ADAS_ERR_INVALID, "bad layer/batch");
    const FileOp& o = e->ops[layer].f;
    Schedule local;
    const char* why = nullptr;
    switch (schedule_at(e, batch, &local).role[layer]) {
    case ROLE_IN_DETECT: why = "is fused into the Detect launch and has no materialised activation (ADAS_NO_DETECT_FUSE=1 keeps it)"; break;
    case ROLE_STEM_INPUT:
    case ROLE_STEM_LEAD: why = "is fused into the stem launch and has no materialised activation (ADAS_NO_STEM=1 keeps it)"; break;
    case ROLE_IN_SHORTCUT_USER: why = "is a projection shortcut computed inside the conv that adds it at this batch (ADAS_NO_DS_FUSE=1 keeps it)"; break;
    case ROLE_IN_CONSUMER_LOADS: why = "is folded into its consumer's loads and has no materialised activation (ADAS_NO_UPSAMPLE_FOLD=1 keeps it)"; break;
    case ROLE_C2F_LEAD:
    case ROLE_C2F_HIDDEN: why = "is computed inside a fused C2f launch: its activation stays in LDS (ADAS_NO_C2F_FUSE=1 keeps it)"; break;
    case ROLE_PAIR_FIRST: why = "is the first conv of a fused 3x3 pair: its activation stays in LDS (ADAS_NO_PAIR_FUSE=1 keeps it)"; break;
    default: break;
    }
    ADAS_REQUIRE(!why, ADAS_ERR_INVALID, "layer %d (%s) %s", layer, e->ops[layer].name.c_str(), why);
    TView v = make_view(e, o.out_buf, o.out_coff, o.out_c);
    if (o.type == OP_INPUT) v.c = 8;
    if (dims) { dims[0] = batch; dims[1] = v.c; dims[2] = v.h; dims[3] = v.w; }
    if (!h_out) return ADAS_OK;
    size_t n = (size_t)batch * v.c * v.h * v.w;
    float* d_tmp = nullptr;
    ADAS_HIP_TRY(hipMalloc((void**)&d_tmp, n * 4));
    hipError_t err = launch_nhwc_to_nchw(v, d_tmp, batch, e->prec, 0);
    if (err == hipSuccess) err = hipMemcpy(h_out, d_tmp, n * 4, hipMemcpyDeviceToHost);
    (void)hipFree(d_tmp);
    if (err != hipSuccess) return hip_fail(err, "fetch_activation", __FILE__, __LINE__);
    return ADAS_OK;
}

}
```

vehicle-cv-adas_amd/csrc/engine.h:

```cpp
#pragma once
#include "common.h"
#include "kernels.h"
#include "conv_ml.h"
#include <map>
#include <string>
#include <vector>

namespace adas {

enum { OP_INPUT = 0, OP_CONV, OP_MAXPOOL, OP_UPSAMPLE2, OP_DETECT_V8, OP_DETECT_V5, OP_LAYERNORM, OP_DWCONV , OP_ATTENTION , OP_AVGPOOL ,
       OP_DEPTH2SPACE , OP_DETECT_V6 ,
       OP_SE_GATE ,
       OP_SCALE , OP_WSUM ,
       OP_SHUFFLE  };

struct FileHeader {
    char magic[8];
    uint32_t version, n_bufs, n_ops, n_outputs, in_c, in_h, in_w, in_cpad;
    uint64_t weights_off, weights_bytes;
    double flops;
    char name[64];
};
static_assert(sizeof(FileHeader) == 128, "FileHeader layout");
struct FileBuf {
    uint32_t h, w, c, flags;
};
struct FileOp {
    uint32_t type, n_in;
    int32_t in_buf[8], in_coff[8], in_c[8];
    int32_t out_buf, out_coff, out_c;
    uint32_t kh, kw, stride, pad, act, res_mode;
    int32_t res_buf, res_coff;
    uint32_t flags, reserved, reserved2;
    uint64_t w_off, w_elems, b_off, b_elems;
    double flops;
    float params[8];
    char name[48];
};
static_assert(sizeof(FileOp) == 280, "FileOp layout");
struct FileOut {
    uint32_t buf, offset, ndim, dims[4];
    char name[32];
    uint32_t pad;
};
static_assert(sizeof(FileOut) == 64, "FileOut layout");

struct EngBuf {
    int h, w, c;
    bool f32;
    void* d;
    int alias_of = -1;
};
struct EngOp {
    FileOp f;
    std::string name;
    size_t w_off = 0, b_off = 0;
    int k = 0, kpad = 0, cout_pad = 0, cin_pad = 0;
    int kernel = 0;
    bool skip = false;
    int fuse_pool = -1;
    int fuse_conv2 = -1;
    int ds_src = -1;
    int ds_user = -1;
    size_t ds_w_off = 0;
    size_t x3h8_w_off = 0;
    bool has_x3h8 = false;
    int halo_bn = 0;
    int up_src = -1;
    int pool3[2] = {-1, -1};
    int pair_b = -1;
    int c2f[3] = {-1, -1, -1};
    int det_src[6] = {-1, -1, -1, -1, -1, -1};
};
enum LayerRole {
    ROLE_OWN = 0,
    ROLE_GROUP_LEAD, ROLE_GROUP_MEMBER,
    ROLE_ML_LEAD, ROLE_ML_MEMBER,
    ROLE_IN_SHORTCUT_USER,
    ROLE_IN_CONSUMER_LOADS,
    ROLE_IN_POOL3,
    ROLE_C2F_LEAD, ROLE_C2F_HIDDEN, ROLE_C2F_TAIL,
    ROLE_PAIR_FIRST, ROLE_IN_PAIR,
    ROLE_IN_DETECT,
    ROLE_STEM_LEAD, ROLE_STEM_INPUT, ROLE_STEM_TAIL,
    ROLE_COUNT
};
inline bool role_launches(int r) {
    return r == ROLE_OWN || r == ROLE_GROUP_LEAD || r == ROLE_ML_LEAD || r == ROLE_C2F_LEAD || r == ROLE_PAIR_FIRST || r == ROLE_STEM_LEAD;
}
struct Step {
    enum Kind { OP, GROUP, ML } kind = OP;
    int lead = -1;
    std::vector<int> members;
    int run = -1;
    MlGroup* group = nullptr;
    MlPlan* plan = nullptr;
    bool folds_shortcut = false;
    int ml_items = 0;
};
struct Schedule {
    std::vector<Step> steps;
    std::vector<int> step_of;
    std::vector<uint8_t> role;
};
struct EngOut {
    uint32_t buf, offset, ndim, dims[4];
    size_t elems;
    std::string name;
};

int engine_forward(struct ::adas_engine* e, const float* d_in, int batch, hipStream_t st, bool packed_in = false);
int engine_prepare(struct ::adas_engine* e, int batch);

}

struct adas_engine {
    int prec = 0, max_batch = 1;
    adas::FileHeader hdr;
    std::string name;
    std::vector<adas::EngBuf> bufs;
    std::vector<adas::EngOp> ops;
    std::vector<adas::EngOut> outs;
    void* d_weights = nullptr;
    float* d_input = nullptr;
    size_t weight_bytes = 0, act_bytes = 0;
    std::vector<hipEvent_t> events;
    hipStream_t last = 0;
    enum Mode { PLAIN, GROUPED, ML } mode = PLAIN;
    std::map<int, adas::Schedule> schedules;
    std::vector<char> buf_aliased;
    float* sink_conf = nullptr;
    int* sink_cls = nullptr;
};

namespace adas {

inline size_t elem_size(const adas_engine* e, const EngBuf& b) { return b.f32 ? 4 : (size_t)prec_esize(e->prec); }

inline TView make_view(const adas_engine* e, int buf, int coff, int c) {
    const EngBuf& b = e->bufs[buf];
    TView v;
    v.p = b.d;
    v.cs = b.c;
    v.coff = coff;
    v.c = c;
    v.h = b.h;
    v.w = b.w;
    v.f32 = b.f32 ? 1 : 0;
    return v;
}

inline TView in_view(const adas_engine* e, const FileOp& o, int k = 0) { return make_view(e, o.in_buf[k], o.in_coff[k], o.in_c[k]); }
inline TView out_view(const adas_engine* e, const FileOp& o) { return make_view(e, o.out_buf, o.out_coff, o.out_c); }

struct Placeholders {
    adas_engine* e;
    bool weights;
    explicit Placeholders(adas_engine* e_) : e(e_), weights(!e_->d_weights) {
        for (size_t bi = 0; bi < e->bufs.size(); ++bi) e->bufs[bi].d = (void*)(uintptr_t)((bi + 1) << 12);
        for (auto& b : e->bufs)
            if (b.alias_of >= 0) b.d = e->bufs[b.alias_of].d;
        if (weights) e->d_weights = (void*)(uintptr_t)((e->bufs.size() + 1) << 12);
    }
    ~Placeholders() {
        for (auto& b : e->bufs) b.d = nullptr;
        if (weights) e->d_weights = nullptr;
    }
};

int free_engine(::adas_engine* e);

ConvArgs conv_args_of(const adas_engine* e, int i, int batch);
void attach_shortcut(const adas_engine* e, int i, ConvArgs* a);
Schedule plan_schedule(const adas_engine* e, int batch, bool fused_launches);
void upload_schedule(const adas_engine* e, int batch, Schedule* s);
void free_schedule(Schedule* s);
const Schedule& schedule_at(const adas_engine* e, int batch, Schedule* local);
void layer_label(const adas_engine* e, const Schedule& s, int layer, int batch, char* name, int cap);
int write_schedule_rows(const adas_engine* e, const Schedule& s, int batch, int32_t* step_of, int32_t* role, char* labels, int cap, int32_t* n_ops,
                        int32_t* n_steps);
bool wants_x3h8_packing(int precision, int kernel, int kh, int kw, int stride, int pad, int res_mode, const TView& in, const TView& out);

}
```

vehicle-cv-adas_amd/csrc/engine_load.cpp:

```cpp
#include "engine.h"
#include <errno.h>
#include <string.h>
#include <memory>
#include <string>
#include <vector>

using namespace adas;

namespace {

struct Source {
    FILE* f = nullptr;
    const unsigned char* mem = nullptr;
    size_t size = 0, pos = 0;
    Source() = default;
    Source(const void* p, size_t bytes) : mem((const unsigned char*)p), size(bytes) {}
    Source(const Source&) = delete;
    ~Source() { if (f) fclose(f); }
    bool open(const char* path) {
        f = fopen(path, "rb");
        if (!f) return false;
        if (fseek(f, 0, SEEK_END) == 0) size = (size_t)ftell(f);
        rewind(f);
        return true;
// ... 317 lines not shown
            e->ops[di].det_src[k] = src[k];
            e->ops[src[k]].skip = true;
        }
    }
}

void fuse_c2f(adas_engine* e, const Uses& u) {
    for (int ai = 0; ai < u.n_ops(); ++ai) {
        const int bi = e->ops[ai].pair_b;
        if (bi < 0) continue;
        const FileOp &qa = u.op(ai), &qb = u.op(bi);
        const int cat = qa.in_buf[0];
        if (qa.in_c[0] != 16 || qb.out_buf != cat || qb.out_coff != qa.in_coff[0] + 16 || qb.res_mode != RES_AFTER_ACT || qa.in_coff[0] < 16 || u.aliased(cat)) continue;
        if (qb.res_buf != cat || qb.res_coff != qa.in_coff[0]) continue;
        int c1 = -1, c2 = -1;
        for (int j = 0; j < u.n_ops(); ++j) {
            const FileOp& q = u.op(j);
            if (q.type != OP_CONV || q.kh != 1 || q.kw != 1 || q.stride != 1 || q.pad != 0 || q.act != ACT_SILU || q.res_mode != RES_NONE || q.n_in != 1 ||
                e->ops[j].skip)
                continue;
            if (j < ai && q.out_buf == cat && q.out_coff == qa.in_coff[0] - 16 && q.out_c == 32 && q.in_c[0] == 32 && e->ops[j].up_src < 0) c1 = j;
            if (j > bi && q.in_buf[0] == cat && q.in_coff[0] == qa.in_coff[0] - 16 && q.in_c[0] == 48 && q.out_c == 32) c2 = j;
        }
        if (c1 < 0 || c2 < 0 || u.readers(cat).count != 3 || u.is_output(cat)) continue;
        bool sole_writers = true;
        for (int j = 0; j < u.n_ops(); ++j) sole_writers = sole_writers && !(u.op(j).out_buf == cat && j != c1 && j != bi);
        if (!sole_writers) continue;
        const FileOp &q1 = u.op(c1), &q2 = u.op(c2);
        bool safe = !(q2.out_buf == q1.in_buf[0] && q2.out_coff < q1.in_coff[0] + q1.in_c[0] && q1.in_coff[0] < q2.out_coff + q2.out_c);
        for (int j = c1 + 1; j < c2 && safe; ++j)
            safe = j == ai || j == bi || !(u.op(j).out_buf == q2.out_buf || u.op(j).out_buf == q1.in_buf[0] || Uses::reads(u.op(j), q2.out_buf));
        if (!safe) continue;
        const EngBuf& xb = e->bufs[q1.in_buf[0]];
        if ((double)e->max_batch * xb.h * xb.w * xb.c * (e->prec == PREC_X3 ? 4.0 : 2.0) >= 2147483648.0) continue;
        const TView vx = in_view(e, q1), v01 = out_view(e, q1), vy1 = in_view(e, qa), vy2 = out_view(e, qb), vcat = in_view(e, q2), vout = out_view(e, q2);
        if (!c2f16_applicable(e->prec, vx, v01, vy1, vy2, vcat, vout) && !c2f16_x3_applicable(e->prec, vx, v01, vy1, vy2, vcat, vout)) continue;
        e->ops[c1].c2f[0] = ai; e->ops[c1].c2f[1] = bi; e->ops[c1].c2f[2] = c2;
        e->ops[ai].skip = true;
        e->ops[c2].skip = true;
    }
}

void release_x3_pairs(adas_engine* e) {
    if (e->prec != PREC_X3) return;
    for (auto& a : e->ops) {
        if (a.pair_b < 0 || a.skip) continue;
        e->ops[a.pair_b].skip = false;
        a.pair_b = -1;
    }
}

struct Arena {
    size_t total = 0;
    size_t take(size_t bytes) {
        const size_t off = total;
        total += (bytes + 255) & ~(size_t)255;
        return off;
    }
};

int layout_arena(adas_engine* e, const char* label) {
    const int prec = e->prec;
    const size_t esz = (size_t)prec_esize(prec);
    std::vector<int> fused(e->ops.size(), -1);
    for (auto& op : e->ops)
        if (op.pair_b >= 0) fused[&op - e->ops.data()] = fused[op.pair_b] = CONV_PAIR;
    for (auto& op : e->ops)
        if (op.c2f[0] >= 0) fused[&op - e->ops.data()] = fused[op.c2f[2]] = CONV_C2F_PW;
    for (auto& op : e->ops)
        for (int k = 0; k < 3 && op.f.type == OP_DETECT_V5; ++k)
            if (op.det_src[k] >= 0) fused[op.det_src[k]] = CONV_DET5;
    Arena arena;
    for (auto& op : e->ops) {
        const FileOp& o = op.f;
        if (o.type == OP_CONV) {
            const int cin = o.in_c[0], cout = o.out_c;
            const bool stem = op.kernel == CONV_STEM, stem2 = op.kernel == CONV_STEM2;
            op.k = o.kh * o.kw * cin;
            op.cout_pad = (cout + 127) / 128 * 128;
            size_t w_bytes;
            if (stem || stem2) {
                op.kpad = stem ? 32 * o.kh : 160;
                op.cin_pad = stem ? 4 : 16;
                w_bytes = stem ? (prec == PREC_X3 ? stem_x3_weight_bytes(o.kh, o.out_c) : stem_weight_bytes(o.kh, o.out_c))
                               : (prec == PREC_X3 ? stem2_x3_weight_bytes() : stem2_weight_bytes());
            } else {
                const TView in = in_view(e, o), out = out_view(e, o);
                const ConvPlan pl = plan_conv(prec, o.kh, o.kw, o.stride, o.pad, e->max_batch, o.res_mode, in, out);
                ADAS_REQUIRE(pl.kernel != CONV_FC || o.res_mode == RES_NONE, ADAS_ERR_FORMAT, "[%s]: layer %s: a Linear layer cannot carry a residual", label,
                             op.name.c_str());
                if (pl.kernel == CONV_HALO) op.halo_bn = plan_halo_bn(e->max_batch, (int)o.stride, in, out);
                op.kpad = pl.kpad;
                op.cin_pad = pl.cin_pad;
                const int fixed = fused[&op - e->ops.data()];
                op.kernel = fixed >= 0 ? fixed : pl.kernel;
                w_bytes = (size_t)op.cout_pad * op.kpad * esz;
                if (fixed == CONV_DET5) w_bytes = det5_weight_bytes(cout / 3, cin);
                else {
                    if (wants_x3h8_packing(prec, pl.kernel, o.kh, o.kw, o.stride, o.pad, o.res_mode, in, out)) {
                        op.has_x3h8 = true;
                        op.x3h8_w_off = arena.take(halo8_x3_weight_bytes(cout, cin));
                    }
                    if (op.ds_user >= 0) op.ds_w_off = arena.take((size_t)cout * cin * esz);
                }
            }
            op.w_off = arena.take(w_bytes);
            op.b_off = arena.take((size_t)op.cout_pad * 4);
        } else if (o.type == OP_LAYERNORM || o.type == OP_DWCONV || o.type == OP_SE_GATE) {
            op.w_off = arena.take((size_t)o.w_elems * 4);
            op.b_off = arena.take((size_t)o.b_elems * 4);
        } else if (o.type == OP_DETECT_V5) {
            op.w_off = arena.take(18 * sizeof(float));
        }
    }
    e->weight_bytes = arena.total;
    return ADAS_OK;
}

void fuse_detect_v8(adas_engine* e, const Uses& u) {
    if (!(prec_is16(e->prec) || e->prec == PREC_X3) || env_on("ADAS_NO_DETECT_FUSE")) return;
    for (int di = 0; di < u.n_ops(); ++di) {
        EngOp& dop = e->ops[di];
        if (dop.f.type != OP_DETECT_V8 || dop.f.n_in != 6) continue;
        int src[6];
        bool ok = detect_sources(e, u, di, 6, src, [&](int k, const EngOp& c) {
            const FileOp& q = c.f;
            return q.kh == 1 && q.kw == 1 && q.stride == 1 && q.act == ACT_NONE && q.res_mode == RES_NONE && c.kernel == CONV_PW && !c.skip &&
                   e->bufs[q.out_buf].f32 && !e->bufs[q.in_buf[0]].f32 && (q.in_c[0] & 7) == 0 && q.out_c == (k % 2 == 0 ? 64u : (uint32_t)dop.f.params[0]);
        });
        for (int l = 1; l < 3 && ok; ++l)
            ok = e->ops[src[2 * l]].f.in_c[0] == e->ops[src[0]].f.in_c[0] && e->ops[src[2 * l + 1]].f.in_c[0] == e->ops[src[1]].f.in_c[0];
        if (ok) {
            const size_t ksb = (e->ops[src[0]].f.in_c[0] + 31) / 32, ksc = (e->ops[src[1]].f.in_c[0] + 31) / 32;
            const size_t ntc = ((size_t)dop.f.params[0] + 15) / 16;
            const size_t frag = e->prec == PREC_X3 ? 2048 : 1024;
            if (ksc > 12 || (4 * ksb + ntc * ksc) * frag + (64 + ntc * 16) * 4 > 150 * 1024) ok = false;
            if (e->prec == PREC_X3)
                for (int k = 0; k < 6 && ok; ++k) {
                    const EngOp& c = e->ops[src[k]];
                    ok = c.kpad == e->ops[src[k % 2]].kpad && (size_t)c.kpad >= (k % 2 ? ksc : ksb) * 32 && (c.kpad & 31) == 0 &&
                         (size_t)c.cout_pad >= (k % 2 ? ntc * 16 : 64);
                }
            if (e->prec == PREC_X3 && ok && (size_t)e->ops[src[1]].kpad / 32 > 12) ok = false;
        }
        if (!ok) continue;
        for (int k = 0; k < 6; ++k) {
            dop.det_src[k] = src[k];
            e->ops[src[k]].skip = true;
        }
    }
}

int plan_engine(adas_engine* e, const char* label) {
    Placeholders ids(e);
    const Uses u{e};
    fuse_stem(e, u);
    link_shortcuts(e, u);
    fold_upsamples(e, u);
    fuse_pool_chains(e);
    fuse_pairs(e, u);
    fuse_detect_v5(e, u);
    fuse_c2f(e, u);
    release_x3_pairs(e);
    const int rc = layout_arena(e, label);
    if (rc == ADAS_OK) fuse_detect_v8(e, u);
    return rc;
}

int upload_bias(adas_engine* e, const EngOp& op, Source& src) {
    std::vector<float> b(op.cout_pad, 0.f);
    if (op.f.b_elems > b.size() || !src.read_at(e->hdr.weights_off + op.f.b_off, b.data(), op.f.b_elems * 4)) return ADAS_ERR_FORMAT;
    return hipMemcpy((unsigned char*)e->d_weights + op.b_off, b.data(), b.size() * 4, hipMemcpyHostToDevice) == hipSuccess ? ADAS_OK : ADAS_ERR_HIP;
}

int upload_op(adas_engine* e, const EngOp& op, Source& src, std::vector<float>& h_stage, float* d_stage) {
    const FileOp& o = op.f;
    const int prec = e->prec;
    unsigned char* base = (unsigned char*)e->d_weights;
    auto read_blob = [&](uint64_t off, uint64_t elems, float* dst) { return src.read_at(e->hdr.weights_off + off, dst, elems * 4); };
    auto to_device = [](void* dst, const void* from, size_t bytes) { return hipMemcpy(dst, from, bytes, hipMemcpyHostToDevice) == hipSuccess; };
    if (o.type == OP_CONV) {
        if (o.w_elems != (uint64_t)o.out_c * op.k || !read_blob(o.w_off, o.w_elems, h_stage.data())) return ADAS_ERR_FORMAT;
        if (!to_device(d_stage, h_stage.data(), o.w_elems * 4)) return ADAS_ERR_HIP;
        if (op.kernel == CONV_STEM || op.kernel == CONV_STEM2) {
            std::vector<uint16_t> frag((op.kernel == CONV_STEM2 ? (prec == PREC_X3 ? stem2_x3_weight_bytes() : stem2_weight_bytes())
                                        : prec == PREC_X3       ? stem_x3_weight_bytes(o.kh, o.out_c)
                                                                : stem_weight_bytes(o.kh, o.out_c)) / 2);
            if (op.kernel == CONV_STEM2 && prec == PREC_X3) stem2_x3_pack_weights(h_stage.data(), frag.data());
            else if (op.kernel == CONV_STEM2) stem2_pack_weights(h_stage.data(), frag.data(), prec);
            else if (prec == PREC_X3) stem_x3_pack_weights(h_stage.data(), o.out_c, o.kh, o.kw, o.in_c[0], e->hdr.in_c, frag.data());
            else stem_pack_weights(h_stage.data(), o.out_c, o.kh, o.kw, o.in_c[0], e->hdr.in_c, frag.data(), prec);
            if (!to_device(base + op.w_off, frag.data(), frag.size() * 2)) return ADAS_ERR_HIP;
            return upload_bias(e, op, src);
        }
        hipError_t pe = op.kernel == CONV_DET5 ? launch_pack_weights_det5(d_stage, base + op.w_off, o.out_c / 3, o.in_c[0], prec, 0)
                        : op.kernel == CONV_C2F_PW ? (prec == PREC_X3 ? launch_pack_weights_c2f_pw_x3(d_stage, base + op.w_off, o.out_c, o.in_c[0], 0)
                                                                       : launch_pack_weights_c2f_pw(d_stage, base + op.w_off, o.out_c, o.in_c[0], prec, 0))
                        : op.kernel == CONV_PAIR ? (prec == PREC_X3 ? launch_pack_weights_pair16_x3(d_stage, base + op.w_off, 0)
                                                                     : launch_pack_weights_pair(d_stage, base + op.w_off, o.out_c, prec, 0))
                        : (op.kernel == CONV_FC || op.kernel == CONV_PW)
                            ? launch_pack_weights_fc(d_stage, base + op.w_off, o.out_c, op.cout_pad, o.in_c[0], op.kpad, prec, 0)
                            : op.kernel == CONV_HALO
                            ? launch_pack_weights_halo(d_stage, base + op.w_off, o.out_c, op.cout_pad, o.in_c[0], op.cin_pad, prec, 0, op.halo_bn)
                            : launch_pack_weights(d_stage, base + op.w_off, o.out_c, op.cout_pad, o.kh * o.kw, o.in_c[0], op.cin_pad, op.kpad, prec, 0);
        if (pe == hipSuccess && op.has_x3h8) pe = launch_pack_weights_h8x3(d_stage, base + op.x3h8_w_off, o.out_c, o.in_c[0], 0);
        if (pe == hipSuccess && op.ds_user >= 0) pe = launch_pack_weights_ds(d_stage, base + op.ds_w_off, o.out_c, o.in_c[0], prec, 0);
        if (pe != hipSuccess || hipDeviceSynchronize() != hipSuccess) return ADAS_ERR_HIP;
        return upload_bias(e, op, src);
    }
    if (o.type == OP_LAYERNORM || o.type == OP_SE_GATE || o.type == OP_DWCONV) {
        if (!read_blob(o.w_off, o.w_elems, h_stage.data())) return ADAS_ERR_FORMAT;
        std::vector<float> wt;
        if (o.type == OP_DWCONV) {
            const size_t C_ = o.out_c, T_ = (size_t)o.kh * o.kw;
            wt.resize(C_ * T_);
            for (size_t c = 0; c < C_; ++c)
                for (size_t t = 0; t < T_; ++t) wt[t * C_ + c] = h_stage[c * T_ + t];
        }
        if (!to_device(base + op.w_off, wt.empty() ? h_stage.data() : wt.data(), o.w_elems * 4)) return ADAS_ERR_HIP;
        if (!read_blob(o.b_off, o.b_elems, h_stage.data())) return ADAS_ERR_FORMAT;
        return to_device(base + op.b_off, h_stage.data(), o.b_elems * 4) ? ADAS_OK : ADAS_ERR_HIP;
    }
    if (o.type == OP_DETECT_V5) {
        float anc[18];
        if (o.w_elems != 18 || !read_blob(o.w_off, 18, anc)) return ADAS_ERR_FORMAT;
        return to_device(base + op.w_off, anc, sizeof(anc)) ? ADAS_OK : ADAS_ERR_HIP;
    }
    return ADAS_OK;
}

int allocate_and_upload(adas_engine* e, Source& src, const char* label) {
    for (auto& b : e->bufs) {
        if (b.alias_of >= 0) continue;
        const size_t bytes = (size_t)e->max_batch * b.h * b.w * b.c * elem_size(e, b);
        if (hipMalloc(&b.d, bytes + 256) != hipSuccess) return hip_fail(hipGetLastError(), "hipMalloc(activation buffer)", __FILE__, __LINE__);
        (void)hipMemset(b.d, 0, bytes + 256);
        e->act_bytes += bytes;
    }
    for (auto& b : e->bufs)
        if (b.alias_of >= 0) b.d = e->bufs[b.alias_of].d;
    if (hipMalloc(&e->d_weights, e->weight_bytes + 256) != hipSuccess) return hip_fail(hipGetLastError(), "hipMalloc(weights)", __FILE__, __LINE__);
    (void)hipMemset(e->d_weights, 0, e->weight_bytes + 256);
    size_t max_w = 0;
    for (auto& op : e->ops) {
        max_w = op.f.w_elems > max_w ? (size_t)op.f.w_elems : max_w;
        max_w = op.f.b_elems > max_w ? (size_t)op.f.b_elems : max_w;
    }
    ADAS_REQUIRE(max_w <= src.size / 4, ADAS_ERR_FORMAT, "[%s]: failed while loading weights (bad blob)", label);
    float* d_stage = nullptr;
    std::vector<float> h_stage(max_w ? max_w : 1);
    if (hipMalloc((void**)&d_stage, max_w * 4 + 256) != hipSuccess) return hip_fail(hipGetLastError(), "hipMalloc(weight staging)", __FILE__, __LINE__);
    int rc = ADAS_OK;
    for (size_t i = 0; i < e->ops.size() && rc == ADAS_OK; ++i) rc = upload_op(e, e->ops[i], src, h_stage, d_stage);
    (void)hipFree(d_stage);
    ADAS_REQUIRE(rc == ADAS_OK, rc, "[%s]: failed while loading weights (%s)", label, rc == ADAS_ERR_HIP ? hipGetErrorString(hipGetLastError()) : "bad blob");
    const size_t in_bytes = (size_t)e->max_batch * e->hdr.in_c * e->hdr.in_h * e->hdr.in_w * 4;
    if (hipMalloc((void**)&e->d_input, in_bytes) != hipSuccess) return hip_fail(hipGetLastError(), "hipMalloc(input staging)", __FILE__, __LINE__);
    return engine_prepare(e, e->max_batch) == ADAS_OK ? ADAS_OK : ADAS_ERR_HIP;
}

bool known_precision(int p) { return p == ADAS_PREC_BF16 || p == ADAS_PREC_FP32 || p == ADAS_PREC_FP16 || p == ADAS_PREC_FP16X3; }

int write_plan_rows(const adas_engine* e, int64_t* rows, int rows_cap, int32_t* n_ops, uint64_t* weight_bytes) {
    if (n_ops) *n_ops = (int32_t)e->ops.size();
    if (weight_bytes) *weight_bytes = e->weight_bytes;
    if (!rows) return ADAS_OK;
    ADAS_REQUIRE(rows_cap >= (int)e->ops.size(), ADAS_ERR_CAPACITY, "engine plan: %zu layers, room for %d", e->ops.size(), rows_cap);
    for (const EngOp& op : e->ops) {
        int64_t* r = rows + (size_t)(&op - e->ops.data()) * ADAS_PLAN_COLS;
        int c = 0;
        r[c++] = op.kernel; r[c++] = op.skip; r[c++] = op.fuse_pool; r[c++] = op.fuse_conv2; r[c++] = op.ds_src; r[c++] = op.ds_user; r[c++] = op.up_src;
        for (int v : op.pool3) r[c++] = v;
        r[c++] = op.pair_b;
        for (int v : op.c2f) r[c++] = v;
        for (int v : op.det_src) r[c++] = v;
        r[c++] = op.halo_bn; r[c++] = op.has_x3h8; r[c++] = op.k; r[c++] = op.kpad; r[c++] = op.cin_pad; r[c++] = op.cout_pad;
        r[c++] = (int64_t)op.w_off; r[c++] = (int64_t)op.b_off; r[c++] = (int64_t)op.ds_w_off; r[c++] = (int64_t)op.x3h8_w_off;
        static_assert(ADAS_PLAN_COLS == 29, "plan row layout (include/adas_hip.h)");
    }
    return ADAS_OK;
}

}

bool adas::wants_x3h8_packing(int precision, int kernel, int kh, int kw, int stride, int pad, int res_mode, const TView& in, const TView& out) {
    return precision == PREC_X3 && kernel != CONV_PW && kernel != CONV_FC &&
           (halo8_x3_shape_ok(kh, kw, stride, pad, in, out) || halo_s2p_x3_shape_ok(kh, kw, stride, pad, res_mode, in, out));
}

extern "C" {

int adas_engine_create(const char* model_path, int precision, int max_batch, adas_engine** out) {
    ADAS_REQUIRE(model_path && out && max_batch > 0, ADAS_ERR_INVALID, "adas_engine_create: bad argument");
    ADAS_REQUIRE(known_precision(precision), ADAS_ERR_INVALID, "unknown precision %d", precision);
    Source src;
    ADAS_REQUIRE(src.open(model_path), ADAS_ERR_IO, "The model path [%s] can't not found! (%s)", model_path, strerror(errno));
    EnginePtr e;
    int rc = read_container(src, model_path, true, precision, max_batch, e);
    if (rc == ADAS_OK) rc = validate_container(e.get(), model_path);
    if (rc == ADAS_OK) rc = plan_engine(e.get(), model_path);
    if (rc == ADAS_OK) rc = allocate_and_upload(e.get(), src, model_path);
    if (rc == ADAS_OK) *out = e.release();
    return rc;
}

int adas_engine_plan(const adas_engine* e, int64_t* rows, int rows_cap, int32_t* n_ops, uint64_t* weight_bytes) {
// ... 36 lines not shown
```

vehicle-cv-adas_amd/csrc/engine_schedule.cpp:

```cpp
#include "engine.h"
#include <stdlib.h>
#include <algorithm>
#include <map>
#include <string>
#include <vector>

namespace adas {

ConvArgs conv_args_of(const adas_engine* e, int i, int batch) {
    const EngOp& op = e->ops[i];
    const FileOp& o = op.f;
    unsigned char* wb = (unsigned char*)e->d_weights;
    ConvArgs a;
    a.in = in_view(e, o);
    a.out = out_view(e, o);
    if (o.res_mode != RES_NONE) a.res = make_view(e, o.res_buf, o.res_coff, o.out_c);
    else { a.res = a.out; a.res.p = nullptr; }
    a.wgt = wb + op.w_off;
    a.bias = (const float*)(wb + op.b_off);
    a.n = batch; a.kh = o.kh; a.kw = o.kw; a.stride = o.stride; a.pad = o.pad; a.act = o.act; a.res_mode = o.res_mode;
    a.k = op.k; a.kpad = op.kpad; a.m = batch * a.out.h * a.out.w; a.max_n = e->max_batch; a.prec = e->prec;
    if (op.has_x3h8) a.wgt_h8x3 = wb + op.x3h8_w_off;
    a.halo_bn = op.halo_bn;
    if (op.up_src >= 0) {
        a.up = in_view(e, e->ops[op.up_src].f);
        a.up_c = (int)e->ops[op.up_src].f.out_c;
    }
    return a;
}

void attach_shortcut(const adas_engine* e, int i, ConvArgs* a) {
    const EngOp& dsop = e->ops[e->ops[i].ds_src];
    unsigned char* wb = (unsigned char*)e->d_weights;
    a->ds_in = in_view(e, dsop.f);
    a->ds_w = wb + dsop.ds_w_off;
    a->ds_bias = (const float*)(wb + dsop.b_off);
}

namespace {

bool folds_shortcut(const adas_engine* e, int ci, int batch) {
    const EngOp& op = e->ops[ci];
    if (op.ds_src < 0 || op.kernel != CONV_HALO) return false;
    const ConvArgs a = conv_args_of(e, ci, batch);
    return conv_route(a) == ConvRoute::H8 && halo8_ds_applicable(a, in_view(e, e->ops[op.ds_src].f));
}

std::vector<uint8_t> base_roles(const adas_engine* e, const std::vector<char>& folds) {
    const int n = (int)e->ops.size();
    std::vector<char> in_c2f(n, 0), c2f_tail(n, 0);
    for (auto& q : e->ops)
        for (int k = 0; k < 3 && q.c2f[0] >= 0; ++k) { in_c2f[q.c2f[k]] = 1; c2f_tail[q.c2f[k]] = k == 2; }
    std::vector<uint8_t> role(n);
    for (int i = 0; i < n; ++i) {
        const EngOp& op = e->ops[i];
        const FileOp& o = op.f;
        const bool conv = o.type == OP_CONV;
        role[i] = conv && op.ds_user >= 0 && folds[op.ds_user]                                ? ROLE_IN_SHORTCUT_USER
                  : op.skip && o.type == OP_UPSAMPLE2                                         ? ROLE_IN_CONSUMER_LOADS
                  : op.skip && o.type == OP_MAXPOOL && (o.kh == 5 || o.kh == 9 || o.kh == 13) ? ROLE_IN_POOL3
                  : conv && op.c2f[0] >= 0                                                    ? ROLE_C2F_LEAD
                  : op.skip && conv && in_c2f[i]                                              ? (c2f_tail[i] ? ROLE_C2F_TAIL : ROLE_C2F_HIDDEN)
                  : op.skip && op.kernel == CONV_PAIR                                         ? ROLE_IN_PAIR
                  : conv && op.pair_b >= 0                                                    ? ROLE_PAIR_FIRST
                  : op.skip && conv && o.kh == 1 && (op.kernel == CONV_PW || op.kernel == CONV_DET5) ? ROLE_IN_DETECT
                  : op.skip                                                                   ? (o.type == OP_INPUT ? ROLE_STEM_INPUT : ROLE_STEM_TAIL)
                  : conv && op.kernel == CONV_STEM && (op.fuse_pool >= 0 || op.fuse_conv2 >= 0) ? ROLE_STEM_LEAD
                                                                                              : ROLE_OWN;
    }
    return role;
}

Step op_step(const adas_engine* e, int i, bool folds) {
    const EngOp& op = e->ops[i];
    Step st;
    st.lead = i;
    st.folds_shortcut = folds;
    st.members.push_back(i);
    auto rides = [&](int j) { if (j >= 0) st.members.push_back(j); };
    if (op.f.type == OP_CONV && op.kernel == CONV_STEM) {
        if (e->ops[0].skip) rides(0);
        rides(op.fuse_pool); rides(op.fuse_conv2);
    }
    if (folds) rides(op.ds_src);
    for (int j : op.pool3) rides(j);
    rides(op.pair_b);
    for (int j : op.c2f) rides(j);
    for (int j : op.det_src) rides(j);
    return st;
}

bool shareable_conv(const adas_engine* e, const std::vector<uint8_t>& role, const std::vector<char>& folds, int i, int batch, ConvArgs* a) {
    const EngOp& op = e->ops[i];
    const FileOp& o = op.f;
    if (role[i] != ROLE_OWN || o.type != OP_CONV || (op.kernel != CONV_HALO && op.kernel != CONV_PW)) return false;
    if (folds[i]) return false;
    auto aliased = [&](int b) { return b >= 0 && b < (int)e->buf_aliased.size() && e->buf_aliased[b]; };
    if (aliased(o.in_buf[0]) || aliased(o.out_buf) || (o.res_mode != RES_NONE && aliased(o.res_buf))) return false;
    if (op.up_src >= 0 && aliased(e->ops[op.up_src].f.in_buf[0])) return false;
    *a = conv_args_of(e, i, batch);
    return true;
}

int env_int(const char* name, int dflt) {
    const char* v = getenv(name);
    return v ? atoi(v) : dflt;
}

template <class Cand, class Emit>
void scan_runs(const std::vector<uint8_t>& role, int min_layers, Cand cand, Emit emit) {
    const int n = (int)role.size();
    int i = 0;
    while (i < n) {
        std::vector<ConvArgs> layers;
        std::vector<int> ops;
        int j = i, last = i;
        for (; j < n; ++j) {
            if (!role_launches(role[j])) continue;
            ConvArgs a;
            if ((int)layers.size() >= ML_MAX_LAYERS || !cand(j, &a)) break;
            layers.push_back(a); ops.push_back(j);
            last = j;
        }
        if ((int)layers.size() >= min_layers) emit(ops, layers);
        i = (layers.empty() ? j : last) + 1;
    }
}

void index_steps(Schedule* s) {
    std::fill(s->step_of.begin(), s->step_of.end(), -1);
    for (size_t k = 0; k < s->steps.size(); ++k)
        for (int m : s->steps[k].members) s->step_of[m] = (int)k;
}

void release_tables(Step* st) {
    ml_group_destroy(st->group);
    ml_plan_destroy(st->plan);
    st->group = nullptr; st->plan = nullptr;
}

void unshare_run(Schedule* s, int run) {
    std::vector<Step> out;
    std::vector<int> layers;
    size_t at = 0;
    for (auto& st : s->steps) {
        if (st.run != run) { out.push_back(st); continue; }
        if (layers.empty()) at = out.size();
        release_tables(&st);
        layers.insert(layers.end(), st.members.begin(), st.members.end());
    }
    std::sort(layers.begin(), layers.end());
    for (size_t k = 0; k < layers.size(); ++k) {
        Step st;
        st.lead = layers[k];
        st.members.push_back(layers[k]);
        out.insert(out.begin() + at + k, st);
        s->role[layers[k]] = ROLE_OWN;
    }
    s->steps.swap(out);
    index_steps(s);
}

}

Schedule plan_schedule(const adas_engine* e, int batch, bool fused_launches) {
    const int n = (int)e->ops.size();
    std::vector<char> folds(n, 0);
    for (int i = 0; i < n; ++i) folds[i] = folds_shortcut(e, i, batch);
    Schedule s;
    s.role = base_roles(e, folds);
    s.step_of.assign(n, -1);
    struct Run { int last; std::vector<Step> steps; };
    std::map<int, Run> runs;
    int n_runs = 0;
    if (fused_launches && e->mode == adas_engine::GROUPED) {
        auto cand = [&](int i, ConvArgs* a) {
// ... 184 lines not shown
```

vehicle-cv-adas_amd/csrc/kernels.h:

```cpp
#pragma once
#include <hip/hip_runtime.h>
#include <stdint.h>

namespace adas {

enum { PREC_BF16 = 0, PREC_FP32 = 1, PREC_FP16 = 2, PREC_X3 = 3 };
inline bool prec_is16(int prec) { return prec == PREC_BF16 || prec == PREC_FP16; }
inline int prec_esize(int prec) { return prec_is16(prec) ? 2 : 4; }
enum { ACT_NONE = 0, ACT_SILU = 1, ACT_RELU = 2, ACT_LEAKY = 3 ,
       ACT_HSWISH = 4 , ACT_HSIGMOID = 5 , ACT_RELU6 = 6  };
enum { RES_NONE = 0, RES_AFTER_ACT = 1, RES_BEFORE_ACT = 2 };

int persist_slots(int which);

struct TView {
    void* p;
    int cs, coff, c;
    int h, w;
    int f32;
};

struct ConvArgs {
    TView in, out, res;
    const void* wgt;
    const float* bias;
    int n;
    int kh, kw, stride, pad, act, res_mode;
    int k, kpad, m;
    int max_n;
    int prec;
    TView up{};
    int up_c = 0;
    TView ds_in{};
    const void* ds_w = nullptr;
    const float* ds_bias = nullptr;
    int halo_bn = 0;
    const void* wgt_h8x3 = nullptr;
};

enum { CONV_GATHER = 0, CONV_HALO = 1, CONV_FC = 2, CONV_STEM = 3, CONV_PW = 4, CONV_STEM2 = 5 ,
       CONV_PAIR = 6 ,
       CONV_C2F_PW = 7 ,
       CONV_DET5 = 8  };
struct ConvPlan {
    int kernel;
    int cin_pad;
    int kpad;
};
ConvPlan plan_conv(int prec, int kh, int kw, int stride, int pad, int max_n, int res_mode, const TView& in, const TView& out);

enum class ConvRoute { IGEMM, PWG, HALO, HALO_RW, S2P, H8, PW, FC,
                       X3_FC, X3_PW, H8X3, S2D_X3, S2P_X3, X3,
                       INVALID };
ConvRoute conv_route(const ConvArgs& a);

bool halo_rw_applicable(const ConvArgs& a);
hipError_t launch_conv_halo_rw(const ConvArgs& a, hipStream_t st);
bool halo_s2p_applicable(const ConvArgs& a);
hipError_t launch_conv_halo_s2p(const ConvArgs& a, hipStream_t st);
bool halo_s2p_x3_shape_ok(int kh, int kw, int stride, int pad, int res_mode, const TView& in, const TView& out);
bool halo_s2p_x3_applicable(const ConvArgs& a);
hipError_t launch_conv_s2p_x3(const ConvArgs& a, hipStream_t st);
bool s2d_x3_fits(const ConvArgs& a);
hipError_t launch_conv_s2d_x3(const ConvArgs& a, hipStream_t st);
struct HaloPlan {
    int SW, NS, TPS, WW, maxpix;
    double eff;
    uint32_t mg_ww, mg_sw;
};
bool plan_halo(int Ho, int Wo, int S, HaloPlan* out, int maxpix_cap = 0, int bm = 0, int policy = 0);
bool plan_halo_sw(int Ho, int Wo, int S, int SW, int maxpix_cap, HaloPlan* out, int bm = 0);
int halo_tile_pixels(const ConvArgs& a);
bool halo8_applicable(const ConvArgs& a);
bool halo8_ds_applicable(const ConvArgs& a, const TView& x);
hipError_t launch_pack_weights_ds(const float* src, void* dst, int cout, int cin, int prec, hipStream_t st);
hipError_t launch_conv_halo8(const ConvArgs& a, hipStream_t st);
bool pair_applicable(int prec, int kh, int kw, int stride, int pad, int act, int res_mode, const TView& x, const TView& t, int kh2, int kw2,
                     int stride2, int pad2, int act2, int res_mode2, const TView& y, const TView& res2);
hipError_t launch_pack_weights_pair(const float* src, void* dst, int c, int prec, hipStream_t st);
hipError_t launch_conv_pair(const TView& x, const TView& y, const void* w1, const float* b1, const void* w2, const float* b2, int n, bool has_res,
                            int prec, hipStream_t st);
bool c2f16_applicable(int prec, const TView& x, const TView& cat01, const TView& y1, const TView& y2, const TView& cat, const TView& out);
hipError_t launch_pack_weights_c2f_pw(const float* src, void* dst, int cout, int cin, int prec, hipStream_t st);
size_t c2f_pw_weight_bytes(int cout, int cin);
bool pair_x3_candidate(int prec, int kh, int kw, int stride, int pad, int act, int res_mode, const TView& x, const TView& t, int kh2, int kw2, int stride2,
                       int pad2, int act2, int res_mode2, const TView& y);
bool c2f16_x3_applicable(int prec, const TView& x, const TView& cat01, const TView& y1, const TView& y2, const TView& cat, const TView& out);
hipError_t launch_pack_weights_pair16_x3(const float* src, void* dst, hipStream_t st);
hipError_t launch_pack_weights_c2f_pw_x3(const float* src, void* dst, int cout, int cin, hipStream_t st);
hipError_t launch_conv_c2f16_x3(const TView& x, const TView& out, const void* const w[4], const float* const b[4], int n, hipStream_t st);
hipError_t launch_conv_c2f16(const TView& x, const TView& out, const void* w_cv1, const float* b_cv1, const void* w_a, const float* b_a, const void* w_b,
                             const float* b_b, const void* w_cv2, const float* b_cv2, int n, int prec, hipStream_t st);
bool pw_applicable(int prec, int kh, int kw, int stride, int pad, int res_mode, const TView& in, const TView& out);
bool pwg_applicable(const ConvArgs& a);
hipError_t launch_conv_pwg(const ConvArgs& a, hipStream_t st);
const char* pwg_kernel_name(int m, int cout);
hipError_t launch_conv_x3(const ConvArgs& a, hipStream_t st);
const char* conv_x3_kernel_name(const ConvArgs& a);
hipError_t launch_pack_weights_x3(const float* src, void* dst, int cout, int cout_pad, int taps, int cin, int cin_pad, int kpad, hipStream_t st);
bool halo8_x3_shape_ok(int kh, int kw, int stride, int pad, const TView& in, const TView& out);
bool halo8_x3_applicable(const ConvArgs& a);
size_t halo8_x3_weight_bytes(int cout, int cin);
hipError_t launch_pack_weights_h8x3(const float* src, void* dst, int cout, int cin, hipStream_t st);
hipError_t launch_conv_halo8_x3(const ConvArgs& a, hipStream_t st);
hipError_t launch_conv(const ConvArgs& a, hipStream_t st);
const char* conv_kernel_name(const ConvArgs& a, bool stem = false);

hipError_t launch_input_nchw(const float* nchw, TView out, int n, int c_true, int prec, hipStream_t st);
hipError_t launch_maxpool(TView in, TView out, int n, int k, int s, int p, int prec, hipStream_t st);
hipError_t launch_avgpool(TView in, TView out, int n, int k, int s, int p, int prec, hipStream_t st);
hipError_t launch_upsample2(TView in, TView out, int n, int prec, hipStream_t st);
bool depth2space_supported(const TView& in, const TView& out);
hipError_t launch_depth2space(TView in, TView out, int n, int prec, hipStream_t st);
hipError_t launch_detect_v6(const TView* ins, float* out, int n, int nc, int A, const int strides[3], hipStream_t st);
hipError_t launch_detect_v6_dfl(const TView* ins, float* out, int n, int nc, int A, const int strides[3], hipStream_t st);
bool sppf_pool3_applicable(int prec, const TView& in, const TView out[3]);
hipError_t launch_sppf_pool3(const TView& in, const TView out[3], int n, int prec, hipStream_t st);
hipError_t launch_detect_v8(const TView* ins, float* out, int n, int nc, int A, const int strides[3], hipStream_t st);
hipError_t launch_detect_v8_fused(const TView* hidden, const void* const* wfrag, const float* const* bias, float* out, int n, int nc, int A,
                                  const int strides[3], int prec, hipStream_t st, float* sink_conf = nullptr, int* sink_cls = nullptr);
hipError_t launch_detect_v8_fused_x3(const TView* hidden, const void* const* wfrag, const float* const* bias, int kt_box, int kt_cls, float* out, int n, int nc,
                                     int A, const int strides[3], hipStream_t st_, float* sink_conf = nullptr, int* sink_cls = nullptr);
bool det5_applicable(int prec, int nc, const TView& in, const TView& logits);
size_t det5_weight_bytes(int no, int cin);
hipError_t launch_pack_weights_det5(const float* src, void* dst, int no, int cin, int prec, hipStream_t st);
hipError_t launch_detect_v5_fused(const TView* hidden, const void* const* wfrag, const float* const* bias, float* out, int n, int nc, int A,
                                  const int strides[3], const float* d_anchors, int prec, hipStream_t st, float* sink_conf = nullptr, int* sink_cls = nullptr);
hipError_t launch_detect_v5(const TView* ins, float* out, int n, int nc, int A, const int strides[3],
                            const float* d_anchors, hipStream_t st);
hipError_t launch_layernorm(const float* in, void* out, const float* gamma, const float* beta, int n, int len, float eps,
                            int prec, hipStream_t st);
hipError_t launch_pack_weights(const float* src, void* dst, int cout, int cout_pad, int taps, int cin, int cin_pad, int kpad,
                               int prec, hipStream_t st);
bool stem_applicable(int prec, int in_c_true, int kh, int kw, int stride, int pad, int act, int res_mode, const TView& out, bool pool,
                     const TView& pool_out);
size_t stem_weight_bytes(int kh, int cout);
size_t stem2_weight_bytes();
void stem2_pack_weights(const float* w_ohwi_32x3x3x16, uint16_t* dst_host, int prec);
bool stem2_applicable(int prec, int kh, int pad, int act, const TView& stem_out, int kh2, int kw2, int stride2, int pad2, int act2, int res_mode2,
                      const TView& out2);
hipError_t launch_conv_stem2(const float* nchw, int n, int c_true, int H, int W, int kh, int pad, const void* wfrag, const float* bias,
                             const TView& stem_out, const void* wfrag2, const float* bias2, const TView& out2, bool packed_in, int prec, hipStream_t st);
void stem_pack_weights(const float* w_ohwi, int cout, int kh, int kw, int cs, int c_true, uint16_t* dst_host, int prec);
bool stem_x3_applicable(int in_c_true, int kh, int kw, int stride, int pad, int act, int res_mode, const TView& out);
size_t stem_x3_weight_bytes(int kh, int cout);
void stem_x3_pack_weights(const float* w_ohwi, int cout, int kh, int kw, int cs, int c_true, uint16_t* dst_host);
hipError_t launch_conv_stem_x3(const float* nchw, int n, int c_true, int H, int W, int kh, int pad, int act, const void* wfrag, const float* bias,
                               const TView& out, hipStream_t st);
bool stem2_x3_applicable(int in_c_true, int kh, int pad, int act, const TView& stem_out, int kh2, int kw2, int stride2, int pad2, int act2, int res_mode2,
                         const TView& out2);
size_t stem2_x3_weight_bytes();
void stem2_x3_pack_weights(const float* w_ohwi_32x3x3x16, uint16_t* dst_host);
hipError_t launch_conv_stem2_x3(const float* nchw, int n, int c_true, int H, int W, int kh, int pad, const void* wfrag, const float* bias,
                                const TView& stem_out, const void* wfrag2, const float* bias2, const TView& out2, hipStream_t st);
bool stem_pool_x3_applicable(int in_c_true, int kh, int kw, int stride, int pad, int act, int res_mode, const TView& conv_out, const TView& pool_out);
hipError_t launch_conv_stem_pool_x3(const float* nchw, int n, int c_true, int H, int W, int pad, const void* wfrag, const float* bias,
                                    const TView& conv_out, const TView& pool_out, hipStream_t st);
hipError_t launch_conv_stem(const float* nchw, int n, int c_true, int H, int W, int kh, int pad, int act, const void* wfrag,
                            const float* bias, const TView& conv_out, bool pool, const TView& pool_out, bool packed_in, int prec, hipStream_t st);
inline int halo_bn(int cout) { return cout <= 16 ? 16 : (cout <= 32 ? 32 : ((cout > 64 && cout <= 96) ? 48 : 64)); }
int plan_halo_bn(int max_n, int stride, const TView& in, const TView& out);
hipError_t launch_pack_weights_halo(const float* src, void* dst, int cout, int cout_pad, int cin, int cin_pad, int prec, hipStream_t st, int bn = 0);
bool pw_x3_applicable(int kh, int kw, int stride, int pad, int res_mode, const TView& in, const TView& out);
hipError_t launch_conv_pw_x3(const ConvArgs& a, hipStream_t st);
bool fc_x3_applicable(int kh, int kw, int stride, const TView& in, const TView& out);
hipError_t launch_fc_x3(const ConvArgs& a, hipStream_t st);
hipError_t launch_pack_weights_fcx3(const float* src, void* dst, int cout, int cout_pad, int cin, int kpad, hipStream_t st);
hipError_t launch_pack_weights_fc(const float* src, void* dst, int cout, int cout_pad, int cin, int kpad, int prec, hipStream_t st);
bool se_gate_supported(const TView& in, const TView& gate, int cr, uint64_t w_elems, uint64_t b_elems);
hipError_t launch_se_gate(const TView& in, const TView& gate, const float* w1, const float* w2, int cr, int act_hidden, int act_gate, int n, int prec, hipStream_t st,
                          const TView* scratch = nullptr);
bool scale_supported(const TView& in, const TView& gate, const TView& out);
hipError_t launch_scale(const TView& in, const TView& gate, const TView& out, int n, int prec, hipStream_t st);
bool shuffle_supported(const TView& in, const TView& out, int groups);
hipError_t launch_shuffle(const TView& in, const TView& out, int groups, int n, int prec, hipStream_t st);
bool wsum_supported(int n_in, const TView* ins, const TView& out);
hipError_t launch_wsum(int n_in, const TView* ins, const float* w, const TView& out, int n, int act, int prec, hipStream_t st);
bool dwconv_supported(int k, int stride, int pad, int res_mode, const TView& in, const TView& out);
hipError_t launch_dwconv(const TView& in, const TView& out, const TView& res, int res_mode, const float* wgt, const float* bias, int n, int k,
                         int stride, int pad, int act, int prec, hipStream_t st);
bool attention_supported(int nh, int kd, int hd, const TView& qkv, const TView& out);
hipError_t launch_attention(const TView& qkv, const TView& out, int n, int nh, int kd, int hd, float scale, int prec, hipStream_t st);
hipError_t launch_nhwc_to_nchw(TView in, float* out, int n, int prec, hipStream_t st);

}
```

Baseline: 5643.

## Add narrow-cout item for halo8 x3 conv with larger pixel tiles

When the last 64-wide output-channel block is at most half full, the halo8 fp16x3 conv now launches that block as a separate narrow item. In it all eight waves cover pixels of a 512-pixel tile, the upper-half waves skip weight loads, and the input window is enlarged within the LDS budget. The remaining full channel blocks still go through the existing shared-tile kernel. This is meant to stop spending MFMA work and weight traffic on padded channels, at the cost of an extra launch and a more complex window-load schedule. The rounding-mode setreg calls around the hi-part conversion are also removed.

After: 5685, median of 6. About the same (+0.7%).

```diff
diff --git a/include/adas_hip.h b/include/adas_hip.h
--- a/include/adas_hip.h
+++ b/include/adas_hip.h
@@ -80,6 +80,7 @@
 int adas_debug_ml_plan(const adas_ml_layer_desc* layers, int n_layers, int batch, int precision, int32_t* deps, int32_t* targets,
                        uint64_t* items, int items_cap, int32_t summary[4]);
 int adas_debug_conv_route(const adas_ml_layer_desc* layer, int batch, int precision, char* name, int name_cap);
+int adas_debug_h8x3_items(const adas_ml_layer_desc* layer, int batch, int narrow, int32_t info[6]);
 #define ADAS_PLAN_COLS 29
 int adas_engine_plan(const adas_engine* e, int64_t* rows, int rows_cap, int32_t* n_ops, uint64_t* weight_bytes);
 int adas_debug_engine_plan(const void* tables, size_t bytes, int precision, int max_batch, int64_t* rows, int rows_cap, int32_t* n_ops,
diff --git a/vehicle-cv-adas_amd/_lib.py b/vehicle-cv-adas_amd/_lib.py
--- a/vehicle-cv-adas_amd/_lib.py
+++ b/vehicle-cv-adas_amd/_lib.py
@@ -185,6 +185,7 @@
     "adas_debug_ml_plan": (C.c_int, [C.POINTER(MlLayerDesc), C.c_int, C.c_int, C.c_int, C.POINTER(C.c_int32), C.POINTER(C.c_int32), C.POINTER(C.c_uint64),
                                      C.c_int, C.POINTER(C.c_int32)]),
     "adas_debug_conv_route": (C.c_int, [C.POINTER(MlLayerDesc), C.c_int, C.c_int, C.c_char_p, C.c_int]),
+    "adas_debug_h8x3_items": (C.c_int, [C.POINTER(MlLayerDesc), C.c_int, C.c_int, C.POINTER(C.c_int32)]),
     "adas_engine_plan": (C.c_int, [_P, C.POINTER(C.c_int64), C.c_int, C.POINTER(C.c_int32), C.POINTER(C.c_uint64)]),
     "adas_debug_engine_plan": (C.c_int, [C.c_char_p, C.c_size_t, C.c_int, C.c_int, C.POINTER(C.c_int64), C.c_int, C.POINTER(C.c_int32), C.POINTER(C.c_uint64)]),
     "adas_engine_schedule": (C.c_int, [_P, C.c_int, C.POINTER(C.c_int32), C.POINTER(C.c_int32), C.c_int, C.POINTER(C.c_int32), C.POINTER(C.c_int32)]),
diff --git a/vehicle-cv-adas_amd/csrc/conv_halo8_x3.hip b/vehicle-cv-adas_amd/csrc/conv_halo8_x3.hip
--- a/vehicle-cv-adas_amd/csrc/conv_halo8_x3.hip
+++ b/vehicle-cv-adas_amd/csrc/conv_halo8_x3.hip
@@ -26,6 +26,7 @@
     uint32_t mg_ww, mg_sw;
     uint32_t mg_img, mg_tps, mg_upt;
     int ntiles, tiles8, ncb, cpw;
+    int cb0;
 };
 
 constexpr int X8_THR = 512;
@@ -39,6 +40,15 @@
 constexpr int X8_SLAB = 9 * 64 * 64;
 constexpr uint32_t X8_OOB = 0xF0000000u;
 constexpr int X8_SLOTS = 32;
+constexpr int NX_BM = 512;
+constexpr int NX_TAP = 64 * 64;
+constexpr int NX_RING = 9 * NX_TAP;
+constexpr int NX_DUMP = 4 * 1024;
+constexpr int NX_NWP = (160 * 1024 - NX_RING - NX_DUMP) / 2 / (8 * 1024);
+constexpr int NX_MAXPIX = NX_NWP * 128;
+constexpr int NX_WIN = NX_MAXPIX * 64;
+constexpr int NX_LDS = 2 * NX_WIN + NX_RING + NX_DUMP;
+static_assert(NX_LDS <= 160 * 1024 && NX_NWP >= X8_NWP, "narrow item: LDS budget");
 
 __host__ __device__ constexpr int x8_look(int mode) { return mode == 2 ? 6 : 4; }
 
@@ -63,10 +73,6 @@
 }
 __device__ __forceinline__ yf32x2 x8_join2(uint32_t h, uint32_t l) {
     return __builtin_convertvector(__builtin_bit_cast(e_f16x2, l), yf32x2) * kX3Down + __builtin_convertvector(__builtin_bit_cast(e_f16x2, h), yf32x2);
-}
-__device__ __forceinline__ void x8_hi_mode(bool flush) {
-    if (flush) __builtin_amdgcn_s_setreg((unsigned short)(1 | (6 << 6) | (1 << 11)), 0u);
-    else __builtin_amdgcn_s_setreg((unsigned short)(1 | (6 << 6) | (1 << 11)), 3u);
 }
 __device__ __forceinline__ uint32_t x8_cvt_hi2(yf32x2 v) {
     uint32_t h;
@@ -105,13 +111,17 @@
 #define H8XP(i)
 #endif
 
-__host__ __device__ constexpr int x8s_issued(bool lo, int k, int nwp) { return ((lo ? k >= 3 : (k >= 0 && k < 3)) ? 1 : 0) + ((k >= 1 && k <= nwp) ? 1 : 0); }
+__host__ __device__ constexpr int x8s_wcount(int k, int nwp) { return (k >= 1 && k <= 5 && k <= nwp) ? 1 + (k <= nwp - 5 ? 1 : 0) : 0; }
+__host__ __device__ constexpr int x8s_wfirst(int k, int nwp) { return (k - 1) + (nwp > 5 ? (k - 1 < nwp - 5 ? k - 1 : nwp - 5) : 0); }
+__host__ __device__ constexpr int x8s_issued(bool lo, int k, int nwp) { return ((lo ? k >= 3 : (k >= 0 && k < 3)) ? 1 : 0) + x8s_wcount(k, nwp); }
 __host__ __device__ constexpr int x8s_allow(bool lo, int k, int nwp) { return x8s_issued(lo, k, nwp) + x8s_issued(lo, k - 1, nwp) + x8s_issued(lo, k - 2, nwp); }
 
-template <int ACT, int MODE, bool LH, bool SH, int NWP>
+template <int ACT, int MODE, bool LH, bool SH, int NWP, bool NARROW = false>
 __global__ __launch_bounds__(X8_THR, 1) void conv_h8x3_kernel(H8XDev a) {
     static_assert(!SH || (MODE == 2 && !LH), "shared weight tiles: one barrier per tap row, whole tiles");
-    static_assert(NWP >= 1 && NWP <= X8_NWP && (SH || NWP == X8_NWP), "window pieces per wave");
+    static_assert(NWP >= 1 && NWP <= (NARROW ? NX_NWP : X8_NWP) && (SH || NWP == X8_NWP), "window pieces per wave");
+    static_assert(!NARROW || SH, "the narrow item exists on the shared-tile stream only");
+    constexpr int BM = NARROW ? NX_BM : X8_BM, WIN = NARROW ? NX_WIN : X8_WIN, TAP = NARROW ? NX_TAP : X8_TAP, WR = 2 * WIN;
     Fp16::enter();
     typedef Fp16::vec8 hvec8;
     constexpr int LOOK = x8_look(MODE);
@@ -121,6 +131,8 @@
     const int wave = __builtin_amdgcn_readfirstlane(tid >> 6);
     const int lrow = lane & 15, kg = lane >> 4;
     const int hb = wave >> 2, grp = wave & 3;
+    const int chb = NARROW ? 0 : hb;
+    const int pxg = NARROW ? hb * 4 + grp : grp;
     const int xcd = blockIdx.x & 7, slot = blockIdx.x >> 3, nslot = gridDim.x >> 3;
     int tiles_here = a.ntiles - xcd * a.tiles8;
     tiles_here = tiles_here < 0 ? 0 : (tiles_here > a.tiles8 ? a.tiles8 : tiles_here);
@@ -137,13 +149,16 @@
     const int gsw[4] = {0, 2, 3, 1};
     const uint32_t wlane = (uint32_t)((lane >> 2) * 64 + (((lane & 3) ^ gsw[(lane >> 4) & 3]) << 4));
     const uint32_t wpiece = (uint32_t)((lane & 3) ^ (((lane >> 4) & 1) << 1)) << 5;
-    const uint32_t wrd = (uint32_t)(X8_WR + hb * 4096 + lrow * 64 + ((kg ^ gsw[(lrow >> 2) & 3]) << 4));
+    const uint32_t wrd = (uint32_t)(WR + chb * 4096 + lrow * 64 + ((kg ^ gsw[(lrow >> 2) & 3]) << 4));
+    const bool wnone = NARROW && hb;
+    const int wdst0 = wnone ? WR + 9 * TAP + grp * 1024 : WR + (NARROW ? grp : wave) * 1024, wdstk = wnone ? 0 : TAP;
+    const uint32_t wvoff = wnone ? X8_OOB : wlane, wsmask = wnone ? 0u : ~0u;
     const uint32_t wlane_h = (uint32_t)((lane >> 2) * 64 + (((lane & 3) ^ gsw[(((lane >> 4) & 1) + 2 * (grp & 1)) & 3]) << 4));
-    const uint32_t wdst_h = (uint32_t)(X8_WR + hb * 4096 + 2048 + grp * 512);
+    const uint32_t wdst_h = (uint32_t)(WR + hb * 4096 + 2048 + grp * 512);
 #ifdef ADAS_H8X_NARROW_ST
-    const uint32_t ch_lane = (uint32_t)((hb * 4 + (kg >> 1)) * 32 + (kg & 1) * 8);
-#else
-    const uint32_t ch_lane = (uint32_t)((hb * 4 + (kg >> 1)) * 32 + (kg & 1) * 16);
+    const uint32_t ch_lane = (uint32_t)((chb * 4 + (kg >> 1)) * 32 + (kg & 1) * 8);
+#else
+    const uint32_t ch_lane = (uint32_t)((chb * 4 + (kg >> 1)) * 32 + (kg & 1) * 16);
 #endif
     const bool has_res = a.res_mode != RES_NONE;
 
@@ -157,12 +172,12 @@
         tile -= t.img * per_img;
         const int strip = a.TPS == 1 ? tile : (int)__umulhi((uint32_t)tile, a.mg_tps);
         t.sx0 = strip * a.SW;
-        t.p0 = (tile - strip * a.TPS) * X8_BM;
+        t.p0 = (tile - strip * a.TPS) * BM;
         t.y_first = (int)(((uint32_t)t.p0 * a.mg_sw) >> 20);
         return t;
     };
     auto win_offset = [&](const Tile& t, int i) {
-        const int y_lastp = (int)(((uint32_t)(t.p0 + X8_BM - 1) * a.mg_sw) >> 20);
+        const int y_lastp = (int)(((uint32_t)(t.p0 + BM - 1) * a.mg_sw) >> 20);
         const int npix = (y_lastp - t.y_first + 3) * a.WW;
         const int pix = (wave + 8 * i) * 16 + (lane >> 2);
         const int wy = (int)(((uint32_t)pix * a.mg_ww) >> 20), wx = pix - wy * a.WW;
@@ -173,7 +188,7 @@
         return (off & m) | (X8_OOB & ~m);
     };
     auto tap00 = [&](const Tile& t, int j) {
-        const int p = t.p0 + (grp * 4 + j) * 16 + lrow;
+        const int p = t.p0 + (pxg * 4 + j) * 16 + lrow;
         const int y = (int)(((uint32_t)p * a.mg_sw) >> 20), xs = p - y * a.SW;
         return (uint32_t)((((y - t.y_first) * a.WW + xs) << 6) | (kg << 4));
     };
@@ -182,20 +197,20 @@
         return v ^ ((v >> 3) & 0x20u);
     };
     auto out_pixel = [&](const Tile& t, int j) {
-        const int p = t.p0 + (grp * 4 + j) * 16 + lrow;
+        const int p = t.p0 + (pxg * 4 + j) * 16 + lrow;
         const int y = (int)(((uint32_t)p * a.mg_sw) >> 20), x = t.sx0 + (p - y * a.SW);
         return (y < a.H && x < a.W) ? (uint32_t)((t.img * a.H + y) * a.W + x) : X8_OOB;
     };
-    auto wgt_base = [&](int cb) { return (uint32_t)(((2 * cb + hb) * a.nck) * X8_SLAB + grp * 1024); };
+    auto wgt_base = [&](int cb) { return (uint32_t)(((2 * cb + chb) * a.nck) * X8_SLAB + grp * 1024); };
     auto load_bias = [&](int cb, float4* b) {
 #pragma unroll
-        for (int i = 0; i < 2; ++i) b[i] = *reinterpret_cast<const float4*>(a.bias + cb * 64 + hb * 32 + i * 16 + kg * 4);
+        for (int i = 0; i < 2; ++i) b[i] = *reinterpret_cast<const float4*>(a.bias + cb * 64 + chb * 32 + i * 16 + kg * 4);
     };
 
-    auto first_cb = [&](int u) { return upt == 1 ? 0 : (u - (int)__umulhi((uint32_t)u, a.mg_upt) * upt) * a.cpw; };
+    auto first_cb = [&](int u) { return NARROW ? a.cb0 : upt == 1 ? 0 : (u - (int)__umulhi((uint32_t)u, a.mg_upt) * upt) * a.cpw; };
     int ti = slot, cb = first_cb(slot), cbi = 0;
     Tile cur = decode(ti);
-    uint32_t gcur[X8_NWP], gnxt[X8_NWP];
+    uint32_t gcur[NX_NWP], gnxt[NX_NWP];
     uint32_t xoff[4][9];
     uint32_t po[4];
 #pragma unroll
@@ -217,7 +232,7 @@
         __builtin_amdgcn_raw_ptr_buffer_load_lds(rin, (ylds_vp)(lds8 + (wave + 8 * i) * 1024), 16, gcur[i], 0, 0, 0);
 #pragma unroll
     for (int t = 0; t < LOOK; ++t)
-        __builtin_amdgcn_raw_ptr_buffer_load_lds(rwg, (ylds_vp)(lds8 + X8_WR + t * X8_TAP + wave * 1024), 16, wlane, wcur + t * 4096, 0, 0);
+        __builtin_amdgcn_raw_ptr_buffer_load_lds(rwg, (ylds_vp)(lds8 + wdst0 + t * wdstk), 16, wvoff, (wcur + t * 4096) & wsmask, 0, 0);
     yf32x4 acc[4][4];
 #pragma unroll
     for (int j = 0; j < 4; ++j) {
@@ -243,7 +258,7 @@
         const int cbn = newtile ? first_cb(has_next ? ti + nslot : ti) : cb + 1;
         const uint32_t ch0 = (uint32_t)(cb * 256) + ch_lane;
 #ifndef ADAS_H8X_NO_TRIM
-        const bool wave_on = cb * 64 + hb * 32 < a.cout;
+        const bool wave_on = cb * 64 + chb * 32 < a.cout;
 #else
         constexpr bool wave_on = true;
 #endif
@@ -266,7 +281,7 @@
             }
             const uint32_t wthis = wcur + (uint32_t)c * X8_SLAB;
             const uint32_t wnext = lastc ? wnxt_item : wthis + X8_SLAB;
-            const uint32_t winr = (uint32_t)(((par + c) & 1) * X8_WIN), winw = X8_WIN - winr;
+            const uint32_t winr = (uint32_t)(((par + c) & 1) * WIN), winw = WIN - winr;
             auto tap = [&](auto kk_c) {
                 constexpr int kk = decltype(kk_c)::value;
                 if (lastc && kk == X8_RES_TAP) load_bias(cbn, biasn);
@@ -277,12 +292,12 @@
 #pragma unroll
                         for (int i = 0; i < 2; ++i) {
 #ifdef ADAS_H8X_NARROW_ST
-                            const uint32_t ri = (cb * 64 + hb * 32 + i * 16 + kg * 4 < a.cout) ? ro + i * 64 : X8_OOB;
+                            const uint32_t ri = (cb * 64 + chb * 32 + i * 16 + kg * 4 < a.cout) ? ro + i * 64 : X8_OOB;
                             const yu32x2 rh = __builtin_bit_cast(yu32x2, __builtin_amdgcn_raw_buffer_load_b64(rres, ri, 0, 0));
                             const yu32x2 rl = __builtin_bit_cast(yu32x2, __builtin_amdgcn_raw_buffer_load_b64(rres, ri + 16, 0, 0));
                             rraw[j][i] = yu32x4{rh.x, rh.y, rl.x, rl.y};
 #else
-                            const uint32_t ri = (cb * 64 + hb * 32 + i * 16 + (kg >> 1) * 8 < a.cout) ? ro + i * 64 : X8_OOB;
+                            const uint32_t ri = (cb * 64 + chb * 32 + i * 16 + (kg >> 1) * 8 < a.cout) ? ro + i * 64 : X8_OOB;
                             rraw[j][i] = __builtin_bit_cast(yu32x4, __builtin_amdgcn_raw_buffer_load_b128(rres, ri, 0, 0));
 #endif
                         }
@@ -291,7 +306,7 @@
                 hvec8 wf[4], xf[4];
                 if (wave_on) {
 #pragma unroll
-                    for (int i = islo ? 2 : 0; i < 4; ++i) wf[i] = *reinterpret_cast<const hvec8*>(lds8 + wrd + kk * X8_TAP + ((SH && islo) ? i - 2 : i) * 1024);
+                    for (int i = islo ? 2 : 0; i < 4; ++i) wf[i] = *reinterpret_cast<const hvec8*>(lds8 + wrd + kk * TAP + ((SH && islo) ? i - 2 : i) * 1024);
 #pragma unroll
                     for (int j = 0; j < 4; ++j) xf[j] = *reinterpret_cast<const hvec8*>(lds8 + xoff[j][kk] + winr);
                 }
@@ -299,7 +314,7 @@
                     if constexpr (islo ? kk >= 3 : kk < 3) {
                         constexpr int kt = (kk + 6) % 9;
                         const uint32_t src = (islo ? wnext : wthis) + (uint32_t)kt * 4096u;
-                        __builtin_amdgcn_raw_ptr_buffer_load_lds(rwg, (ylds_vp)(lds8 + X8_WR + kt * X8_TAP + wave * 1024), 16, wlane, src, 0, 0);
+                        __builtin_amdgcn_raw_ptr_buffer_load_lds(rwg, (ylds_vp)(lds8 + wdst0 + kt * wdstk), 16, wvoff, src & wsmask, 0, 0);
                     }
                 } else {
                     constexpr int kt = (kk + LOOK) % 9;
@@ -307,13 +322,16 @@
                     const uint32_t src = (kk + LOOK < 9 ? wthis : wnext) + (uint32_t)kt * 4096u;
                     if (LH && tgt_lo) {
                         if (lane < 32)
-                            __builtin_amdgcn_raw_ptr_buffer_load_lds(rwg, (ylds_vp)(lds8 + wdst_h + kt * X8_TAP), 16, wlane_h, src + 2048u - (uint32_t)grp * 512u, 0, 0);
+                            __builtin_amdgcn_raw_ptr_buffer_load_lds(rwg, (ylds_vp)(lds8 + wdst_h + kt * TAP), 16, wlane_h, src + 2048u - (uint32_t)grp * 512u, 0, 0);
                     } else {
-                        __builtin_amdgcn_raw_ptr_buffer_load_lds(rwg, (ylds_vp)(lds8 + X8_WR + kt * X8_TAP + wave * 1024), 16, wlane, src, 0, 0);
+                        __builtin_amdgcn_raw_ptr_buffer_load_lds(rwg, (ylds_vp)(lds8 + WR + kt * TAP + wave * 1024), 16, wlane, src, 0, 0);
                     }
                 }
-                if constexpr (kk >= 1 && kk <= NWP)
-                    __builtin_amdgcn_raw_ptr_buffer_load_lds(rin, (ylds_vp)(lds8 + winw + (wave + 8 * (kk - 1)) * 1024), 16, lastc ? gnxt[kk - 1] : gcur[kk - 1], 0, 0, 0);
+#pragma unroll
+                for (int q = 0; q < x8s_wcount(kk, NWP); ++q) {
+                    constexpr int p0 = x8s_wfirst(kk, NWP);
+                    __builtin_amdgcn_raw_ptr_buffer_load_lds(rin, (ylds_vp)(lds8 + winw + (wave + 8 * (p0 + q)) * 1024), 16, lastc ? gnxt[p0 + q] : gcur[p0 + q], 0, 0, 0);
+                }
                 constexpr bool sync_here = MODE != 2 || kk % 3 == 2;
                 constexpr int allow = SH ? x8s_allow(islo, kk, NWP) : x8_allow(MODE, kk);
                 constexpr bool with_res = kk >= X8_RES_TAP && (MODE == 2 ? kk / 3 == X8_RES_TAP / 3 : kk < X8_RES_TAP + 3);
@@ -338,7 +356,8 @@
                 if (lastc) {
 #pragma unroll
                     for (int j = 0; j < 4; ++j) xoff[j][kk] = tap_offset(apn[j], kk);
-                    if constexpr (kk < NWP) gnxt[kk] = win_offset(nxt, kk);
+#pragma unroll
+                    for (int q = 0; q < x8s_wcount(kk + 1, NWP); ++q) gnxt[x8s_wfirst(kk + 1, NWP) + q] = win_offset(nxt, x8s_wfirst(kk + 1, NWP) + q);
                 }
                 if (wave_on) {
 #pragma unroll
@@ -402,7 +421,6 @@
                     acc[i + 2][j] = yf32x4{0.f, 0.f, 0.f, 0.f};
                 }
             uint32_t hw[4][2][2];
-            x8_hi_mode(true);
 #pragma unroll
             for (int j = 0; j < 4; ++j)
 #pragma unroll
@@ -410,13 +428,12 @@
                     hw[j][i][0] = x8_cvt_hi2(val[j][i][0]);
                     hw[j][i][1] = x8_cvt_hi2(val[j][i][1]);
                 }
-            x8_hi_mode(false);
 #pragma unroll
             for (int j = 0; j < 4; ++j) {
                 const uint32_t oo = po[j] == X8_OOB ? X8_OOB : (po[j] * (uint32_t)a.out_cs + (uint32_t)a.out_coff) * 4u + ch0;
 #pragma unroll
                 for (int i = 0; i < 2; ++i) {
-                    const uint32_t oi = (cb * 64 + hb * 32 + i * 16 + (kg >> 1) * 8 < a.cout) ? oo + i * 64 : X8_OOB;
+                    const uint32_t oi = (cb * 64 + chb * 32 + i * 16 + (kg >> 1) * 8 < a.cout) ? oo + i * 64 : X8_OOB;
                     const uint32_t l0 = x8_lo2(val[j][i][0], hw[j][i][0]), l1 = x8_lo2(val[j][i][1], hw[j][i][1]);
                     const auto s0 = __builtin_amdgcn_permlane16_swap(hw[j][i][0], l0, false, false);
                     const auto s1 = __builtin_amdgcn_permlane16_swap(hw[j][i][1], l1, false, false);
@@ -433,9 +450,9 @@
 #pragma unroll
                 for (int i = 0; i < 2; ++i) {
 #ifdef ADAS_H8X_NARROW_ST
-                    const uint32_t oi = (cb * 64 + hb * 32 + i * 16 + kg * 4 < a.cout) ? oo + i * 64 : X8_OOB;
-#else
-                    const uint32_t oi = (cb * 64 + hb * 32 + i * 16 + (kg >> 1) * 8 < a.cout) ? oo + i * 64 : X8_OOB;
+                    const uint32_t oi = (cb * 64 + chb * 32 + i * 16 + kg * 4 < a.cout) ? oo + i * 64 : X8_OOB;
+#else
+                    const uint32_t oi = (cb * 64 + chb * 32 + i * 16 + (kg >> 1) * 8 < a.cout) ? oo + i * 64 : X8_OOB;
 #endif
                     float v[4];
 #pragma unroll
@@ -550,6 +567,7 @@
     return v;
 }
 static bool x8_plan(int Ho, int Wo, HaloPlan* pl) { return plan_halo(Ho, Wo, 1, pl, X8_MAXPIX, 0, x8_policy()); }
+static bool nx_plan(int Ho, int Wo, HaloPlan* pl) { return plan_halo(Ho, Wo, 1, pl, NX_MAXPIX, NX_BM, x8_policy()) && pl->eff >= 0.6 && pl->maxpix <= NX_MAXPIX; }
 
 static double x8_min_fill() {
     static double v = -1.0;
@@ -639,21 +657,35 @@
     return v != 0;
 }
 
-template <int NWP>
+template <int NWP, bool NARROW = false>
 static hipError_t x8_launch_sh(const H8XDev& d, int act, dim3 grid, hipStream_t st) {
     static bool attr_done = false;
     if (!attr_done) {
-        (void)hipFuncSetAttribute((const void*)conv_h8x3_kernel<ACT_NONE, 2, false, true, NWP>, hipFuncAttributeMaxDynamicSharedMemorySize, 160 * 1024);
-        (void)hipFuncSetAttribute((const void*)conv_h8x3_kernel<ACT_SILU, 2, false, true, NWP>, hipFuncAttributeMaxDynamicSharedMemorySize, 160 * 1024);
-        (void)hipFuncSetAttribute((const void*)conv_h8x3_kernel<ACT_RELU, 2, false, true, NWP>, hipFuncAttributeMaxDynamicSharedMemorySize, 160 * 1024);
-        (void)hipFuncSetAttribute((const void*)conv_h8x3_kernel<ACT_LEAKY, 2, false, true, NWP>, hipFuncAttributeMaxDynamicSharedMemorySize, 160 * 1024);
+        (void)hipFuncSetAttribute((const void*)conv_h8x3_kernel<ACT_NONE, 2, false, true, NWP, NARROW>, hipFuncAttributeMaxDynamicSharedMemorySize, 160 * 1024);
+        (void)hipFuncSetAttribute((const void*)conv_h8x3_kernel<ACT_SILU, 2, false, true, NWP, NARROW>, hipFuncAttributeMaxDynamicSharedMemorySize, 160 * 1024);
+        (void)hipFuncSetAttribute((const void*)conv_h8x3_kernel<ACT_RELU, 2, false, true, NWP, NARROW>, hipFuncAttributeMaxDynamicSharedMemorySize, 160 * 1024);
+        (void)hipFuncSetAttribute((const void*)conv_h8x3_kernel<ACT_LEAKY, 2, false, true, NWP, NARROW>, hipFuncAttributeMaxDynamicSharedMemorySize, 160 * 1024);
         attr_done = true;
     }
-    if (act == ACT_SILU) hipLaunchKernelGGL((conv_h8x3_kernel<ACT_SILU, 2, false, true, NWP>), grid, dim3(X8_THR), X8_LDS, st, d);
-    else if (act == ACT_RELU) hipLaunchKernelGGL((conv_h8x3_kernel<ACT_RELU, 2, false, true, NWP>), grid, dim3(X8_THR), X8_LDS, st, d);
-    else if (act == ACT_LEAKY) hipLaunchKernelGGL((conv_h8x3_kernel<ACT_LEAKY, 2, false, true, NWP>), grid, dim3(X8_THR), X8_LDS, st, d);
-    else hipLaunchKernelGGL((conv_h8x3_kernel<ACT_NONE, 2, false, true, NWP>), grid, dim3(X8_THR), X8_LDS, st, d);
+    constexpr int lds = NARROW ? NX_LDS : X8_LDS;
+    if (act == ACT_SILU) hipLaunchKernelGGL((conv_h8x3_kernel<ACT_SILU, 2, false, true, NWP, NARROW>), grid, dim3(X8_THR), lds, st, d);
+    else if (act == ACT_RELU) hipLaunchKernelGGL((conv_h8x3_kernel<ACT_RELU, 2, false, true, NWP, NARROW>), grid, dim3(X8_THR), lds, st, d);
+    else if (act == ACT_LEAKY) hipLaunchKernelGGL((conv_h8x3_kernel<ACT_LEAKY, 2, false, true, NWP, NARROW>), grid, dim3(X8_THR), lds, st, d);
+    else hipLaunchKernelGGL((conv_h8x3_kernel<ACT_NONE, 2, false, true, NWP, NARROW>), grid, dim3(X8_THR), lds, st, d);
     return hipGetLastError();
+}
+
+bool halo8_x3_narrow(const ConvArgs& a, HaloPlan* pn) {
+    const int rem = a.out.c % 64, ncb = x8_cout_pad(a.out.c) / 64;
+    if (rem < 1 || rem > 32 || !x8_share() || x8_mode() == 3) return false;
+    int on = a.h8x_narrow;
+    if (on < 0) { const char* e = getenv("ADAS_H8X_NARROW"); on = e ? atoi(e) : 1; }
+    HaloPlan pw;
+    if (on < (ncb > 1 ? 2 : 1) || !nx_plan(a.out.h, a.out.w, pn) || !x8_plan(a.out.h, a.out.w, &pw)) return false;
+    const long nt = (long)a.n * pn->NS * pn->TPS;
+    if (nt * pn->NS * pn->TPS >= (1L << 32) || x8_blocks_per_unit((nt + 7) / 8, 1) <= 0) return false;
+    const long ntw = (long)a.n * pw.NS * pw.TPS;
+    return ncb == 1 || x8_blocks_per_unit((ntw + 7) / 8, ncb - 1) > 0;
 }
 
 template <int MODE, bool LH>
@@ -685,6 +717,8 @@
             if (x8_blocks_per_unit((nt + 7) / 8, x8_cout_pad(a.out.c) / 64) > 0) pl = alt;
         }
     }
+    HaloPlan pn;
+    const bool narrow = halo8_x3_narrow(a, &pn);
     H8XDev d;
     d.in = a.in.p; d.wgt = a.wgt_h8x3; d.bias = a.bias; d.out = a.out.p; d.res = a.res.p;
     d.in_cs = a.in.cs; d.in_coff = a.in.coff; d.cin = a.in.c; d.H = a.in.h; d.W = a.in.w;
@@ -695,22 +729,40 @@
     d.wgt_bytes = (uint32_t)halo8_x3_weight_bytes(a.out.c, a.in.c);
     d.out_bytes = (uint32_t)((size_t)a.n * a.out.h * a.out.w * a.out.cs * 4);
     d.res_bytes = a.res_mode != RES_NONE ? (uint32_t)((size_t)a.n * a.out.h * a.out.w * a.res.cs * 4) : 0u;
-    d.SW = pl.SW; d.NS = pl.NS; d.TPS = pl.TPS; d.WW = pl.WW;
-    d.mg_ww = pl.mg_ww; d.mg_sw = pl.mg_sw;
-    d.mg_img = (uint32_t)(((1ull << 32) + (uint64_t)(pl.NS * pl.TPS) - 1) / (uint64_t)(pl.NS * pl.TPS));
-    d.mg_tps = (uint32_t)(((1ull << 32) + (uint64_t)pl.TPS - 1) / (uint64_t)pl.TPS);
-    d.ntiles = a.n * pl.NS * pl.TPS;
-    d.tiles8 = (d.ntiles + 7) / 8;
-    d.ncb = x8_cout_pad(a.out.c) / 64;
-    d.cpw = x8_blocks_per_unit(d.tiles8, d.ncb);
-    if (d.cpw <= 0) return hipErrorInvalidValue;
-    const int upt = d.ncb / d.cpw;
-    d.mg_upt = (uint32_t)(((1ull << 32) + (uint64_t)upt - 1) / (uint64_t)upt);
-    const int units8 = d.tiles8 * upt;
     static int max_slots = -1;
     if (max_slots < 0) { const char* e = getenv("ADAS_H8X_SLOTS"); max_slots = e ? atoi(e) : X8_SLOTS; if (max_slots < 8 || max_slots > 4096) max_slots = X8_SLOTS; }
-    const int slots = units8 < max_slots ? units8 : max_slots;
-    dim3 grid(8 * slots);
+    dim3 grid;
+    auto lay_out = [&](const HaloPlan& p, int ncb, int cb0) {
+        d.SW = p.SW; d.NS = p.NS; d.TPS = p.TPS; d.WW = p.WW;
+        d.mg_ww = p.mg_ww; d.mg_sw = p.mg_sw;
+        d.mg_img = (uint32_t)(((1ull << 32) + (uint64_t)(p.NS * p.TPS) - 1) / (uint64_t)(p.NS * p.TPS));
+        d.mg_tps = (uint32_t)(((1ull << 32) + (uint64_t)p.TPS - 1) / (uint64_t)p.TPS);
+        d.ntiles = a.n * p.NS * p.TPS;
+        d.tiles8 = (d.ntiles + 7) / 8;
+        d.ncb = ncb; d.cb0 = cb0;
+        d.cpw = x8_blocks_per_unit(d.tiles8, d.ncb);
+        if (d.cpw <= 0) return false;
+        const int upt = d.ncb / d.cpw;
+        d.mg_upt = (uint32_t)(((1ull << 32) + (uint64_t)upt - 1) / (uint64_t)upt);
+        const int units8 = d.tiles8 * upt;
+        grid = dim3(8 * (units8 < max_slots ? units8 : max_slots));
+        return true;
+    };
+    const int ncb_all = x8_cout_pad(a.out.c) / 64;
+    if (narrow) {
+        if (ncb_all > 1) {
+            if (!lay_out(pl, ncb_all - 1, 0)) return hipErrorInvalidValue;
+            const int nwp = (pl.maxpix + 127) / 128;
+            const hipError_t err = nwp <= 3 ? x8_launch_sh<3>(d, a.act, grid, st) : nwp == 4 ? x8_launch_sh<4>(d, a.act, grid, st) : x8_launch_sh<5>(d, a.act, grid, st);
+            if (err != hipSuccess) return err;
+        }
+        if (!lay_out(pn, 1, ncb_all - 1)) return hipErrorInvalidValue;
+        const int nwp = (pn.maxpix + 127) / 128;
+        if (nwp <= 5) return x8_launch_sh<5, true>(d, a.act, grid, st);
+        if (nwp == 6) return x8_launch_sh<6, true>(d, a.act, grid, st);
+        return x8_launch_sh<7, true>(d, a.act, grid, st);
+    }
+    if (!lay_out(pl, ncb_all, 0)) return hipErrorInvalidValue;
     const int forced = x8_mode();
     const bool pingpong = forced == 3;
     if (x8_share() && forced != 3) {
diff --git a/vehicle-cv-adas_amd/csrc/engine.cpp b/vehicle-cv-adas_amd/csrc/engine.cpp
--- a/vehicle-cv-adas_amd/csrc/engine.cpp
+++ b/vehicle-cv-adas_amd/csrc/engine.cpp
@@ -408,6 +408,21 @@
     return ADAS_OK;
 }
 
+int adas_debug_h8x3_items(const adas_ml_layer_desc* layer, int batch, int narrow, int32_t info[6]) {
+    ADAS_REQUIRE(layer && batch > 0 && info, ADAS_ERR_INVALID, "adas_debug_h8x3_items: bad argument");
+    ConvArgs a = conv_args_of_desc(*layer, batch, PREC_X3);
+    const ConvPlan pl = plan_conv(PREC_X3, a.kh, a.kw, a.stride, a.pad, a.max_n, a.res_mode, a.in, a.out);
+    a.kpad = pl.kpad;
+    if (wants_x3h8_packing(PREC_X3, pl.kernel, a.kh, a.kw, a.stride, a.pad, a.res_mode, a.in, a.out)) a.wgt_h8x3 = (const void*)(uintptr_t)0x1000;
+    ADAS_REQUIRE(conv_route(a) == ConvRoute::H8X3, ADAS_ERR_INVALID, "adas_debug_h8x3_items: the layer launches on %s at batch %d", conv_kernel_name(a), batch);
+    a.h8x_narrow = narrow;
+    HaloPlan pn{};
+    for (int i = 0; i < 6; ++i) info[i] = 0;
+    if (!halo8_x3_narrow(a, &pn)) return ADAS_OK;
+    info[0] = 1; info[1] = pn.SW; info[2] = pn.NS; info[3] = pn.TPS; info[4] = pn.maxpix; info[5] = (a.out.c + 63) / 64 - 1;
+    return ADAS_OK;
+}
+
 int adas_engine_precision(const adas_engine* e) { return e ? e->prec : -1; }
 int adas_engine_model_io_half(const adas_engine* e) { return e ? (int)((e->hdr.in_cpad >> 16) & 1u) : 0; }
 
diff --git a/vehicle-cv-adas_amd/csrc/engine.h b/vehicle-cv-adas_amd/csrc/engine.h
--- a/vehicle-cv-adas_amd/csrc/engine.h
+++ b/vehicle-cv-adas_amd/csrc/engine.h
@@ -128,6 +128,7 @@
     hipStream_t last = 0;
     enum Mode { PLAIN, GROUPED, ML } mode = PLAIN;
     std::map<int, adas::Schedule> schedules;
+    int h8x_narrow = 1;
     std::vector<char> buf_aliased;
     float* sink_conf = nullptr;
     int* sink_cls = nullptr;
diff --git a/vehicle-cv-adas_amd/csrc/engine_load.cpp b/vehicle-cv-adas_amd/csrc/engine_load.cpp
--- a/vehicle-cv-adas_amd/csrc/engine_load.cpp
+++ b/vehicle-cv-adas_amd/csrc/engine_load.cpp
@@ -493,6 +493,7 @@
 }
 
 int plan_engine(adas_engine* e, const char* label) {
+    { const char* v = getenv("ADAS_H8X_NARROW"); e->h8x_narrow = v ? atoi(v) : 1; if (e->h8x_narrow < 0 || e->h8x_narrow > 2) e->h8x_narrow = 1; }
     Placeholders ids(e);
     const Uses u{e};
     fuse_stem(e, u);
diff --git a/vehicle-cv-adas_amd/csrc/engine_schedule.cpp b/vehicle-cv-adas_amd/csrc/engine_schedule.cpp
--- a/vehicle-cv-adas_amd/csrc/engine_schedule.cpp
+++ b/vehicle-cv-adas_amd/csrc/engine_schedule.cpp
@@ -22,6 +22,7 @@
     a.k = op.k; a.kpad = op.kpad; a.m = batch * a.out.h * a.out.w; a.max_n = e->max_batch; a.prec = e->prec;
     if (op.has_x3h8) a.wgt_h8x3 = wb + op.x3h8_w_off;
     a.halo_bn = op.halo_bn;
+    a.h8x_narrow = e->h8x_narrow;
     if (op.up_src >= 0) {
         a.up = in_view(e, e->ops[op.up_src].f);
         a.up_c = (int)e->ops[op.up_src].f.out_c;
diff --git a/vehicle-cv-adas_amd/csrc/kernels.h b/vehicle-cv-adas_amd/csrc/kernels.h
--- a/vehicle-cv-adas_amd/csrc/kernels.h
+++ b/vehicle-cv-adas_amd/csrc/kernels.h
@@ -36,6 +36,7 @@
     const float* ds_bias = nullptr;
     int halo_bn = 0;
     const void* wgt_h8x3 = nullptr;
+    int h8x_narrow = -1;
 };
 
 enum { CONV_GATHER = 0, CONV_HALO = 1, CONV_FC = 2, CONV_STEM = 3, CONV_PW = 4, CONV_STEM2 = 5 ,
@@ -100,6 +101,7 @@
 hipError_t launch_pack_weights_x3(const float* src, void* dst, int cout, int cout_pad, int taps, int cin, int cin_pad, int kpad, hipStream_t st);
 bool halo8_x3_shape_ok(int kh, int kw, int stride, int pad, const TView& in, const TView& out);
 bool halo8_x3_applicable(const ConvArgs& a);
+bool halo8_x3_narrow(const ConvArgs& a, HaloPlan* narrow_plan);
 size_t halo8_x3_weight_bytes(int cout, int cin);
 hipError_t launch_pack_weights_h8x3(const float* src, void* dst, int cout, int cin, hipStream_t st);
 hipError_t launch_conv_halo8_x3(const ConvArgs& a, hipStream_t st);
```
